# pangenome/poasta

Measured on AMD Instinct MI355X. Metric: Gcells/sec (aligned bases/sec in config), gap-affine POA alignment, 1k-node POA x 10k x 1 kbp queries per GPU, higher is better.
Workload: dtype u16

## Files before the change

include/poasta_amd.h:

```cpp
#ifndef POASTA_AMD_H
#define POASTA_AMD_H

#include <stdint.h>

#ifdef __cplusplus
extern "C" {
#endif

#define POA_NONE 0xFFFFFFFFu
#define POA_SCORE_UNVISITED 0xFFFFFFFFu

#define POA_OK 0
#define POA_ERR_INVALID_ARG (-1)
#define POA_ERR_NOT_A_DAG (-2)
#define POA_ERR_NO_DEVICE (-3)
#define POA_ERR_HIP (-4)
#define POA_ERR_CAPACITY (-5)
#define POA_ERR_OUT_OF_MEMORY (-6)
#define POA_ERR_UNSUPPORTED (-7)

#define POA_FLAG_AMBIGUOUS 0x01u
#define POA_FLAG_START_QUIRK 0x02u
#define POA_FLAG_REF_PANIC 0x04u
#define POA_FLAG_SHORT_QUERY 0x08u
// ... 175 lines not shown
#define POA_LAYOUT_DERIVED_GAPS 8u
#define POA_LAYOUT_RELATIVE 4u
int poa_batch_last_layout(poa_batch_t* b, uint32_t* layout);
int poa_batch_band_info(poa_batch_t* b, uint32_t out[4]);
enum {
    POA_KERNEL_NONE = 0,
    POA_KERNEL_FORWARD,
    POA_KERNEL_PACKED,
    POA_KERNEL_PX,
    POA_KERNEL_PXMW,
    POA_KERNEL_BAND
};
#define POA_LAUNCH_FUSE 1u
#define POA_LAUNCH_MW 2u
int poa_batch_last_launch(poa_batch_t* b, uint32_t chunk, uint32_t out[8]);
int poa_batch_band_pair_info(poa_batch_t* b, uint32_t out[4]);
#define POA_BAND_PAIR_MASK 3
#define POA_BAND_PAIR_RULE 2
#define POA_BAND_NARROW_SHIFT 2
int poa_batch_band_narrow_info(poa_batch_t* b, uint32_t out[4]);
int poa_batch_fetch_planes(poa_batch_t* b, uint32_t query, uint32_t* m, uint32_t* i, uint32_t* d);
int poa_batch_fetch_compact(poa_batch_t* b, uint32_t query, uint16_t* m_raw, uint16_t* d, uint8_t* d_kept);
int poa_batch_fetch_planes_2piece(poa_batch_t* b, uint32_t query, uint32_t* m, uint32_t* i1, uint32_t* d1, uint32_t* i2, uint32_t* d2);
void poa_batch_destroy(poa_batch_t* b);

typedef struct poa_multi poa_multi_t;
int poa_multi_footprint(const poa_graph_t* const* graphs, uint32_t n_graphs, const uint64_t* graph_qoff,
                        const uint64_t* qoff, const poa_config_t* cfg, uint64_t* bytes, uint64_t* largest_query_bytes);
int poa_multi_create(const poa_graph_t* const* graphs, uint32_t n_graphs, const uint64_t* graph_qoff, int device,
                     const uint8_t* qseq, const uint64_t* qoff, const poa_config_t* cfg, uint64_t workspace_bytes,
                     poa_multi_t** out);
int poa_multi_run(poa_multi_t* m, const poa_costs_t* costs, const poa_config_t* cfg, void* stream);
int poa_multi_fetch(poa_multi_t* m, uint32_t* score, poa_aln_pair_t* pairs, uint64_t* pair_off, uint64_t pair_capacity,
                    uint32_t* flags, poa_stats_t* stats);
int poa_multi_stats(poa_multi_t* m, poa_stats_t* stats);
int poa_multi_device_results(poa_multi_t* m, void** score, void** flags, void** pair_off, void** pairs);
int poa_multi_workspace_bytes(poa_multi_t* m, uint64_t* bytes);
void poa_multi_destroy(poa_multi_t* m);
int poa_align_multi(const poa_graph_t* const* graphs, uint32_t n_graphs, const uint64_t* graph_qoff,
                    const poa_costs_t* costs, const poa_config_t* cfg, const uint8_t* qseq, const uint64_t* qoff,
                    uint32_t* score, poa_aln_pair_t* pairs, uint64_t* pair_off, uint64_t pair_capacity, uint32_t* flags,
                    poa_stats_t* stats, int device);

int poa_multi_footprint_2piece(const poa_graph_t* const* graphs, uint32_t n_graphs, const uint64_t* graph_qoff,
                               const uint64_t* qoff, const poa_config_t* cfg, uint64_t* bytes, uint64_t* largest_query_bytes);
int poa_multi_create_2piece(const poa_graph_t* const* graphs, uint32_t n_graphs, const uint64_t* graph_qoff, int device,
                            const uint8_t* qseq, const uint64_t* qoff, const poa_config_t* cfg, uint64_t workspace_bytes,
                            poa_multi_t** out);
int poa_multi_run_2piece(poa_multi_t* m, const poa_costs2_t* costs, const poa_config_t* cfg, void* stream);
int poa_align_multi_2piece(const poa_graph_t* const* graphs, uint32_t n_graphs, const uint64_t* graph_qoff,
                           const poa_costs2_t* costs, const poa_config_t* cfg, const uint8_t* qseq, const uint64_t* qoff,
                           uint32_t* score, poa_aln_pair_t* pairs, uint64_t* pair_off, uint64_t pair_capacity,
                           uint32_t* flags, poa_stats_t* stats, int device);

typedef struct poa_scoreset poa_scoreset_t;
int poa_scoreset_footprint(const poa_graph_t* const* graphs, uint32_t n_graphs, uint32_t n_queries, const uint64_t* qoff,
                           uint64_t n_pairs, const uint32_t* pair_query, const uint32_t* pair_graph, const poa_config_t* cfg,
                           uint64_t* bytes, uint64_t* largest_pair_bytes);
int poa_scoreset_create(const poa_graph_t* const* graphs, uint32_t n_graphs, int device, uint32_t n_queries, const uint8_t* qseq,
                        const uint64_t* qoff, uint64_t n_pairs, const uint32_t* pair_query, const uint32_t* pair_graph,
                        const poa_config_t* cfg, uint64_t workspace_bytes, poa_scoreset_t** out);
int poa_scoreset_run(poa_scoreset_t* s, const poa_costs_t* costs, const poa_config_t* cfg, void* stream);
int poa_scoreset_run_2piece(poa_scoreset_t* s, const poa_costs2_t* costs, const poa_config_t* cfg, void* stream);
int poa_scoreset_fetch(poa_scoreset_t* s, uint32_t* score, uint32_t* flags, poa_stats_t* stats);
int poa_scoreset_stats(poa_scoreset_t* s, poa_stats_t* stats);
int poa_scoreset_device_results(poa_scoreset_t* s, void** score, void** flags);
int poa_scoreset_workspace_bytes(poa_scoreset_t* s, uint64_t* bytes);
void poa_scoreset_destroy(poa_scoreset_t* s);
int poa_score_pairs(const poa_graph_t* const* graphs, uint32_t n_graphs, const poa_costs_t* costs, const poa_config_t* cfg,
                    uint32_t n_queries, const uint8_t* qseq, const uint64_t* qoff, uint64_t n_pairs, const uint32_t* pair_query,
                    const uint32_t* pair_graph, uint32_t* score, uint32_t* flags, poa_stats_t* stats, int device);
int poa_score_pairs_2piece(const poa_graph_t* const* graphs, uint32_t n_graphs, const poa_costs2_t* costs, const poa_config_t* cfg,
                           uint32_t n_queries, const uint8_t* qseq, const uint64_t* qoff, uint64_t n_pairs,
                           const uint32_t* pair_query, const uint32_t* pair_graph, uint32_t* score, uint32_t* flags,
                           poa_stats_t* stats, int device);

#ifdef __cplusplus
}
#endif
#include "poasta_amd_scoreset_cap.h"
#include "poasta_amd_scoreset_best.h"
#include "poasta_amd_tb.h"
#include "poasta_amd_multi_dense.h"
#endif
```

poasta_amd/_lib.py:

```python
import ctypes as C
import os
import subprocess

_HERE = os.path.dirname(os.path.abspath(__file__))
LIB_PATH = os.environ.get("POA_LIB_PATH") or os.path.join(_HERE, "libpoasta_amd.so")
CSRC = os.path.join(_HERE, "csrc")

POA_OK = 0
ERRORS = {-1: "POA_ERR_INVALID_ARG", -2: "POA_ERR_NOT_A_DAG", -3: "POA_ERR_NO_DEVICE", -4: "POA_ERR_HIP",
          -5: "POA_ERR_CAPACITY", -6: "POA_ERR_OUT_OF_MEMORY", -7: "POA_ERR_UNSUPPORTED"}
POA_NONE = 0xFFFFFFFF
FLAG_AMBIGUOUS, FLAG_START_QUIRK, FLAG_REF_PANIC, FLAG_SHORT_QUERY, FLAG_TRUNCATED, FLAG_EMPTY_GRAPH = 1, 2, 4, 8, 16, 32
FLAG_CAPPED = 0x80

EXPORTS = ["poa_version", "poa_last_error", "poa_device_count", "poa_graph_create", "poa_graph_destroy",
           "poa_graph_rows", "poa_graph_node_rows", "poa_graph_update", "poa_align_batch", "poa_align_batch_ex", "poa_align_batch_2piece", "poa_align_batch_2piece_ex", "poa_planes_2piece", "poa_release_cache", "poa_batch_create", "poa_batch_run",
           "poa_batch_run_ex",
           "poa_batch_fetch", "poa_batch_stats", "poa_batch_device_results", "poa_batch_fetch_search_counters", "poa_batch_last_layout", "poa_batch_band_info", "poa_batch_band_pair_info", "poa_batch_band_narrow_info", "poa_batch_last_launch", "poa_batch_fetch_planes", "poa_batch_fetch_compact", "poa_batch_destroy",
           "poa_batch_run_2piece", "poa_batch_fetch_planes_2piece",
           "poa_graph_sweep_slots", "poa_batch_create_ex", "poa_batch_workspace_bytes", "poa_graph_checkpoint_plan", "poa_graph_checkpoint_plan2",
           "poa_multi_footprint", "poa_multi_create", "poa_multi_run", "poa_multi_fetch", "poa_multi_stats", "poa_multi_device_results",
           "poa_multi_workspace_bytes", "poa_multi_destroy", "poa_align_multi",
           "poa_multi_footprint_2piece", "poa_multi_create_2piece", "poa_multi_run_2piece", "poa_align_multi_2piece",
           "poa_scoreset_footprint", "poa_scoreset_create", "poa_scoreset_run", "poa_scoreset_run_2piece", "poa_scoreset_fetch",
           "poa_scoreset_stats", "poa_scoreset_device_results", "poa_scoreset_workspace_bytes", "poa_scoreset_destroy",
           "poa_score_pairs", "poa_score_pairs_2piece",
           "poa_graph_sweep_checks"]
EXPORTS_SCORESET_CAP = ["poa_scoreset_run_capped", "poa_scoreset_run_2piece_capped", "poa_scoreset_fetch_swept"]
EXPORTS_SCORESET_BEST = ["poa_scoreset_run_best", "poa_scoreset_run_2piece_best", "poa_scoreset_fetch_best", "poa_scoreset_device_best",
                         "poa_score_best", "poa_score_best_2piece"]
CFG_BEST_PAIR_ORDER = 2
EXPORTS_TB = ["poa_batch_tb_info"]
TB_LEAN_SHIFT = 4
EXPORTS_MULTI_DENSE = ["poa_multi_footprint_dense", "poa_multi_create_dense", "poa_multi_run_dense", "poa_align_multi_dense",
                       "poa_graph_compact_elems", "poa_multi_last_launch"]


class PoaBest(C.Structure):
    _fields_ = [("pair", C.c_uint32), ("score", C.c_uint32), ("flags", C.c_uint32), ("second_score", C.c_uint32),
                ("n_within", C.c_uint32), ("reserved", C.c_uint32 * 3)]


class PoaCosts2(C.Structure):
    _fields_ = [("mismatch", C.c_uint8), ("gap_open1", C.c_uint8), ("gap_extend1", C.c_uint8), ("gap_open2", C.c_uint8),
                ("gap_extend2", C.c_uint8), ("wide_planes", C.c_uint8), ("reserved", C.c_uint8 * 2)]


class PoaCosts(C.Structure):
    _fields_ = [("mismatch", C.c_uint8), ("gap_open", C.c_uint8), ("gap_extend", C.c_uint8), ("reserved", C.c_uint8)]


class PoaBound(C.Structure):
    _fields_ = [("kind", C.c_uint32), ("value", C.c_uint32)]


class PoaConfig(C.Structure):
    _fields_ = [("mode", C.c_uint32), ("heuristic", C.c_uint32), ("pruning", C.c_uint32), ("queue_entries_per_cell", C.c_float),
                ("flags", C.c_uint32), ("span", C.c_uint32), ("qry_free_begin", PoaBound), ("qry_free_end", PoaBound),
                ("graph_free_begin", PoaBound), ("graph_free_end", PoaBound), ("tune", C.c_uint32 * 32)]


TUNE_KEYS = ("PLANES", "COMPACT", "PACKED", "RELATIVE", "PX", "MF", "MW", "PXMW", "FWD_QUADS", "FUSE_TB", "TB_GROUP", "TB_DEPTH",
             "EXACT_IMPL", "EXACT_LANES", "EXACT_LDS", "WS_LANES", "WS_GROUP", "WS_WAVES", "WS_RING_GLOBAL", "WS_STATIC",
             "WS_CHUNK_CAP", "WS_PROF", "PS_LANES", "PS_LEAN", "TIMING", "WS_ADAPT", "WS_REC", "CKPT_ROWS", "BAND", "BAND_DELTA", "BAND_PAIR", "CAP_STRIDE")
EXACT_IMPLS = {"lane": 1, "wave": 2, "flat": 3}


def tune_from_env(cfg=None, **overrides):
    vals = {}
    for i, k in enumerate(TUNE_KEYS):
        v = overrides.get(k.lower(), os.environ.get("POA_" + k))
        if v is None or v == "":
            continue
        vals[i] = EXACT_IMPLS[v] if (k == "EXACT_IMPL" and v in EXACT_IMPLS) else int(v)
    nv = overrides.get("band_narrow", os.environ.get("POA_BAND_NARROW"))
    if nv is not None and nv != "":
        i = TUNE_KEYS.index("BAND_PAIR")
        vals[i] = (min(vals[i], 1) if i in vals else 2) | ((2 if int(nv) else 1) << 2)
    lv = overrides.get("tb_lean", os.environ.get("POA_TB_LEAN"))
    if lv is not None and lv != "":
        i = TUNE_KEYS.index("BAND_PAIR")
        vals[i] = (vals[i] if i in vals else 2) | ((2 if int(lv) else 1) << TB_LEAN_SHIFT)
    if cfg is None:
        if not vals:
            return None
        cfg = PoaConfig()
    for i, v in vals.items():
        cfg.tune[i] = v + 1
    return cfg


BOUND_UNBOUNDED, BOUND_INCLUDED, BOUND_EXCLUDED = 0, 1, 2
SPAN_GLOBAL, SPAN_ENDS_FREE = 0, 1


MODE_DENSE, MODE_EXACT, MODE_HYBRID, MODE_SCORE, MODE_CHECKPOINT, MODE_CHECKPOINT2 = 0, 1, 2, 3, 4, 5
HEURISTIC_DIJKSTRA, HEURISTIC_MINGAP = 0, 1
FLAG_EXACT_OVERFLOW = 0x40
CFG_FULL_PLANES = 1


class PoaStats(C.Structure):
    _fields_ = [("cells", C.c_uint64), ("bases", C.c_uint64), ("plane_bytes", C.c_uint64), ("n_queries", C.c_uint32),
                ("n_chunks", C.c_uint32), ("n_forward_launches", C.c_uint32), ("n_flagged", C.c_uint32),
                ("ms_forward", C.c_float), ("ms_traceback", C.c_float), ("ms_h2d", C.c_float), ("ms_d2h", C.c_float),
                ("ms_exact", C.c_float), ("n_exact", C.c_uint32), ("ms_total", C.c_float), ("n_runs", C.c_uint32)]

    def as_dict(self):
        return {k: getattr(self, k) for k, _ in self._fields_ }


class PoaError(RuntimeError):
    def __init__(self, code, msg):
        super().__init__("%s (%d): %s" % (ERRORS.get(code, "POA_ERR"), code, msg))
        self.code = code


def build(force=False):
    srcs = [os.path.join(CSRC, f) for f in os.listdir(CSRC)] + [os.path.join(_HERE, "..", "include", h) for h in ("poasta_amd.h", "poasta_amd_scoreset_cap.h", "poasta_amd_scoreset_best.h", "poasta_amd_tb.h", "poasta_amd_multi_dense.h")]
    stale = not os.path.exists(LIB_PATH) or any(os.path.getmtime(s) > os.path.getmtime(LIB_PATH) for s in srcs)
    if force or stale:
        subprocess.check_call(["make", "-C", CSRC] + (["-B"] if force else []))
    return LIB_PATH


_lib = None


def lib():
    global _lib
    if _lib is not None:
        return _lib
    if not os.path.exists(LIB_PATH):
        raise ImportError("poasta_amd: %s is missing — build it with `python -c 'import __graft_entry__ as g; g.build()'` "
                          "(hipcc --offload-arch=gfx950). There is no CPU fallback." % LIB_PATH)
    L = C.CDLL(LIB_PATH)
    vp = C.c_void_p
    L.poa_version.restype = C.c_char_p
    L.poa_last_error.restype = C.c_char_p
    L.poa_device_count.restype = C.c_int
    L.poa_graph_create.restype = C.c_int
    L.poa_graph_create.argtypes = [C.c_uint32, C.c_uint32, C.c_uint32, vp, vp, vp, vp, vp, C.POINTER(vp)]
    L.poa_graph_destroy.argtypes = [vp]
    L.poa_graph_destroy.restype = None
    L.poa_graph_rows.restype = C.c_uint32
    L.poa_graph_rows.argtypes = [vp]
    L.poa_graph_node_rows.restype = C.c_int
    L.poa_graph_node_rows.argtypes = [vp, vp]
    L.poa_align_batch.restype = C.c_int
    L.poa_align_batch.argtypes = [vp, C.POINTER(PoaCosts), C.c_uint32, vp, vp, vp, vp, vp, C.c_uint64, vp,
                                  C.POINTER(PoaStats), C.c_int]
    L.poa_align_batch_ex.restype = C.c_int
    L.poa_align_batch_ex.argtypes = [vp, C.POINTER(PoaCosts), C.POINTER(PoaConfig), C.c_uint32, vp, vp, vp, vp, vp, C.c_uint64, vp,
                                     C.POINTER(PoaStats), C.c_int]
    L.poa_align_batch_2piece.restype = C.c_int
    L.poa_align_batch_2piece.argtypes = [vp, C.POINTER(PoaCosts2), C.c_uint32, vp, vp, vp, vp, vp, C.c_uint64, vp,
                                         C.POINTER(PoaStats), C.c_int]
    L.poa_align_batch_2piece_ex.restype = C.c_int
    L.poa_align_batch_2piece_ex.argtypes = [vp, C.POINTER(PoaCosts2), C.POINTER(PoaConfig), C.c_uint32, vp, vp, vp, vp, vp, C.c_uint64, vp,
                                            C.POINTER(PoaStats), vp, C.c_int]
    L.poa_planes_2piece.restype = C.c_int
    L.poa_planes_2piece.argtypes = [vp, C.POINTER(PoaCosts2), vp, C.c_uint32, vp, vp, vp, vp, vp, C.c_int]
    L.poa_batch_run_ex.restype = C.c_int
    L.poa_batch_run_ex.argtypes = [vp, C.POINTER(PoaCosts), C.POINTER(PoaConfig), vp]
    L.poa_batch_create.restype = C.c_int
    L.poa_batch_create.argtypes = [vp, C.c_int, C.c_uint32, vp, vp, C.c_uint64, C.POINTER(vp)]
    L.poa_graph_sweep_slots.restype = C.c_int
    L.poa_graph_sweep_slots.argtypes = [vp, vp, vp]
    if hasattr(L, "poa_graph_sweep_checks"):
        L.poa_graph_sweep_checks.restype = C.c_int
        L.poa_graph_sweep_checks.argtypes = [vp, C.c_uint32, vp, vp]
        L.poa_scoreset_run_capped.restype = C.c_int
        L.poa_scoreset_run_capped.argtypes = [vp, C.POINTER(PoaCosts), C.POINTER(PoaConfig), vp, vp]
        L.poa_scoreset_run_2piece_capped.restype = C.c_int
        L.poa_scoreset_run_2piece_capped.argtypes = [vp, C.POINTER(PoaCosts2), C.POINTER(PoaConfig), vp, vp]
        L.poa_scoreset_fetch_swept.restype = C.c_int
        L.poa_scoreset_fetch_swept.argtypes = [vp, vp]
    if hasattr(L, "poa_scoreset_run_best"):
        L.poa_scoreset_run_best.restype = C.c_int
        L.poa_scoreset_run_best.argtypes = [vp, C.POINTER(PoaCosts), C.POINTER(PoaConfig), C.c_uint32, vp, vp]
        L.poa_scoreset_run_2piece_best.restype = C.c_int
        L.poa_scoreset_run_2piece_best.argtypes = [vp, C.POINTER(PoaCosts2), C.POINTER(PoaConfig), C.c_uint32, vp, vp]
        L.poa_scoreset_fetch_best.restype = C.c_int
        L.poa_scoreset_fetch_best.argtypes = [vp, vp]
        L.poa_scoreset_device_best.restype = C.c_int
        L.poa_scoreset_device_best.argtypes = [vp, C.POINTER(vp)]
        L.poa_score_best.restype = C.c_int
        L.poa_score_best.argtypes = [vp, C.c_uint32, C.POINTER(PoaCosts), C.POINTER(PoaConfig), C.c_uint32, vp, vp, C.c_uint64, vp, vp,
                                     C.c_uint32, vp, vp, vp, vp, C.POINTER(PoaStats), C.c_int]
        L.poa_score_best_2piece.restype = C.c_int
        L.poa_score_best_2piece.argtypes = [vp, C.c_uint32, C.POINTER(PoaCosts2), C.POINTER(PoaConfig), C.c_uint32, vp, vp, C.c_uint64, vp, vp,
                                            C.c_uint32, vp, vp, vp, vp, C.POINTER(PoaStats), C.c_int]
    L.poa_graph_checkpoint_plan.restype = C.c_int
    L.poa_graph_checkpoint_plan.argtypes = [vp, C.c_uint32, vp, vp, vp]
    L.poa_graph_checkpoint_plan2.restype = C.c_int
    L.poa_graph_checkpoint_plan2.argtypes = [vp, C.c_uint32, vp, vp, vp]
    L.poa_batch_create_ex.restype = C.c_int
    L.poa_batch_create_ex.argtypes = [vp, C.c_int, C.c_uint32, vp, vp, C.POINTER(PoaConfig), C.c_uint64, C.POINTER(vp)]
    L.poa_batch_workspace_bytes.restype = C.c_int
    L.poa_batch_workspace_bytes.argtypes = [vp, C.POINTER(C.c_uint64)]
    L.poa_batch_run.restype = C.c_int
    L.poa_batch_run.argtypes = [vp, C.POINTER(PoaCosts), vp]
    L.poa_batch_fetch.restype = C.c_int
    L.poa_batch_fetch.argtypes = [vp, vp, vp, vp, C.c_uint64, vp, C.POINTER(PoaStats)]
    L.poa_batch_stats.restype = C.c_int
    L.poa_batch_stats.argtypes = [vp, C.POINTER(PoaStats)]
    L.poa_batch_fetch_search_counters.restype = C.c_int
    L.poa_batch_fetch_search_counters.argtypes = [vp, vp]
    L.poa_batch_last_layout.restype = C.c_int
    L.poa_batch_last_layout.argtypes = [vp, vp]
    if hasattr(L, "poa_batch_band_info"):
        L.poa_batch_band_info.restype = C.c_int
        L.poa_batch_band_info.argtypes = [vp, vp]
    if hasattr(L, "poa_batch_band_pair_info"):
        L.poa_batch_band_pair_info.restype = C.c_int
        L.poa_batch_band_pair_info.argtypes = [vp, vp]
    if hasattr(L, "poa_batch_band_narrow_info"):
        L.poa_batch_band_narrow_info.restype = C.c_int
        L.poa_batch_band_narrow_info.argtypes = [vp, vp]
    if hasattr(L, "poa_batch_tb_info"):
        L.poa_batch_tb_info.restype = C.c_int
        L.poa_batch_tb_info.argtypes = [vp, vp]
    if hasattr(L, "poa_batch_last_launch"):
        L.poa_batch_last_launch.restype = C.c_int
        L.poa_batch_last_launch.argtypes = [vp, C.c_uint32, vp]
    L.poa_batch_device_results.restype = C.c_int
    L.poa_batch_device_results.argtypes = [vp, C.POINTER(vp), C.POINTER(vp), C.POINTER(vp), C.POINTER(vp)]
    L.poa_batch_fetch_planes.restype = C.c_int
    L.poa_batch_fetch_planes.argtypes = [vp, C.c_uint32, vp, vp, vp]
    if hasattr(L, "poa_batch_fetch_compact"):
        L.poa_batch_fetch_compact.restype = C.c_int
        L.poa_batch_fetch_compact.argtypes = [vp, C.c_uint32, vp, vp, vp]
    L.poa_batch_run_2piece.restype = C.c_int
    L.poa_batch_run_2piece.argtypes = [vp, C.POINTER(PoaCosts2), C.POINTER(PoaConfig), vp]
    L.poa_batch_fetch_planes_2piece.restype = C.c_int
    L.poa_batch_fetch_planes_2piece.argtypes = [vp, C.c_uint32, vp, vp, vp, vp, vp]
    L.poa_batch_destroy.argtypes = [vp]
    L.poa_batch_destroy.restype = None
    L.poa_multi_footprint.restype = C.c_int
    L.poa_multi_footprint.argtypes = [vp, C.c_uint32, vp, vp, C.POINTER(PoaConfig), C.POINTER(C.c_uint64), C.POINTER(C.c_uint64)]
    L.poa_multi_create.restype = C.c_int
    L.poa_multi_create.argtypes = [vp, C.c_uint32, vp, C.c_int, vp, vp, C.POINTER(PoaConfig), C.c_uint64, C.POINTER(vp)]
    L.poa_multi_run.restype = C.c_int
    L.poa_multi_run.argtypes = [vp, C.POINTER(PoaCosts), C.POINTER(PoaConfig), vp]
    L.poa_multi_fetch.restype = C.c_int
    L.poa_multi_fetch.argtypes = [vp, vp, vp, vp, C.c_uint64, vp, C.POINTER(PoaStats)]
    L.poa_multi_stats.restype = C.c_int
    L.poa_multi_stats.argtypes = [vp, C.POINTER(PoaStats)]
    L.poa_multi_device_results.restype = C.c_int
    L.poa_multi_device_results.argtypes = [vp, C.POINTER(vp), C.POINTER(vp), C.POINTER(vp), C.POINTER(vp)]
    L.poa_multi_workspace_bytes.restype = C.c_int
    L.poa_multi_workspace_bytes.argtypes = [vp, C.POINTER(C.c_uint64)]
    L.poa_multi_destroy.argtypes = [vp]
    L.poa_multi_destroy.restype = None
    L.poa_align_multi.restype = C.c_int
    L.poa_align_multi.argtypes = [vp, C.c_uint32, vp, C.POINTER(PoaCosts), C.POINTER(PoaConfig), vp, vp, vp, vp, vp, C.c_uint64, vp,
                                  C.POINTER(PoaStats), C.c_int]
    L.poa_multi_footprint_2piece.restype = C.c_int
    L.poa_multi_footprint_2piece.argtypes = L.poa_multi_footprint.argtypes
    L.poa_multi_create_2piece.restype = C.c_int
    L.poa_multi_create_2piece.argtypes = L.poa_multi_create.argtypes
    L.poa_multi_run_2piece.restype = C.c_int
    L.poa_multi_run_2piece.argtypes = [vp, C.POINTER(PoaCosts2), C.POINTER(PoaConfig), vp]
    L.poa_align_multi_2piece.restype = C.c_int
    L.poa_align_multi_2piece.argtypes = [vp, C.c_uint32, vp, C.POINTER(PoaCosts2), C.POINTER(PoaConfig), vp, vp, vp, vp, vp, C.c_uint64, vp,
                                         C.POINTER(PoaStats), C.c_int]
    if hasattr(L, "poa_multi_create_dense"):
        L.poa_multi_footprint_dense.restype = C.c_int
        L.poa_multi_footprint_dense.argtypes = L.poa_multi_footprint.argtypes
        L.poa_multi_create_dense.restype = C.c_int
        L.poa_multi_create_dense.argtypes = L.poa_multi_create.argtypes
        L.poa_multi_run_dense.restype = C.c_int
        L.poa_multi_run_dense.argtypes = L.poa_multi_run.argtypes
        L.poa_align_multi_dense.restype = C.c_int
        L.poa_align_multi_dense.argtypes = L.poa_align_multi.argtypes
        L.poa_graph_compact_elems.restype = C.c_int
        L.poa_graph_compact_elems.argtypes = [vp, C.c_uint32, C.POINTER(C.c_uint64)]
        L.poa_multi_last_launch.restype = C.c_int
        L.poa_multi_last_launch.argtypes = [vp, C.c_uint32, vp]
    L.poa_scoreset_footprint.restype = C.c_int
    L.poa_scoreset_footprint.argtypes = [vp, C.c_uint32, C.c_uint32, vp, C.c_uint64, vp, vp, C.POINTER(PoaConfig), C.POINTER(C.c_uint64),
                                         C.POINTER(C.c_uint64)]
    L.poa_scoreset_create.restype = C.c_int
    L.poa_scoreset_create.argtypes = [vp, C.c_uint32, C.c_int, C.c_uint32, vp, vp, C.c_uint64, vp, vp, C.POINTER(PoaConfig), C.c_uint64,
                                      C.POINTER(vp)]
    L.poa_scoreset_run.restype = C.c_int
    L.poa_scoreset_run.argtypes = [vp, C.POINTER(PoaCosts), C.POINTER(PoaConfig), vp]
    L.poa_scoreset_run_2piece.restype = C.c_int
    L.poa_scoreset_run_2piece.argtypes = [vp, C.POINTER(PoaCosts2), C.POINTER(PoaConfig), vp]
    L.poa_scoreset_fetch.restype = C.c_int
    L.poa_scoreset_fetch.argtypes = [vp, vp, vp, C.POINTER(PoaStats)]
    L.poa_scoreset_stats.restype = C.c_int
    L.poa_scoreset_stats.argtypes = [vp, C.POINTER(PoaStats)]
    L.poa_scoreset_device_results.restype = C.c_int
    L.poa_scoreset_device_results.argtypes = [vp, C.POINTER(vp), C.POINTER(vp)]
    L.poa_scoreset_workspace_bytes.restype = C.c_int
    L.poa_scoreset_workspace_bytes.argtypes = [vp, C.POINTER(C.c_uint64)]
    L.poa_scoreset_destroy.argtypes = [vp]
    L.poa_scoreset_destroy.restype = None
    L.poa_score_pairs.restype = C.c_int
    L.poa_score_pairs.argtypes = [vp, C.c_uint32, C.POINTER(PoaCosts), C.POINTER(PoaConfig), C.c_uint32, vp, vp, C.c_uint64, vp, vp, vp, vp,
                                  C.POINTER(PoaStats), C.c_int]
    L.poa_score_pairs_2piece.restype = C.c_int
    L.poa_score_pairs_2piece.argtypes = [vp, C.c_uint32, C.POINTER(PoaCosts2), C.POINTER(PoaConfig), C.c_uint32, vp, vp, C.c_uint64, vp, vp,
                                         vp, vp, C.POINTER(PoaStats), C.c_int]
# ... 8 lines not shown
```

poasta_amd/aligner.py:

```python
import ctypes as C
import os

import numpy as np

from . import _lib
from .graph import FlatGraph, pack_queries


class GapAffine:

    def __init__(self, cost_mismatch, cost_gap_extend, cost_gap_open):
        for v in (cost_mismatch, cost_gap_extend, cost_gap_open):
            if not 0 <= int(v) <= 255:
                raise ValueError("GapAffine costs are u8")
        self.cost_mismatch, self.cost_gap_extend, self.cost_gap_open = int(cost_mismatch), int(cost_gap_extend), int(cost_gap_open)

    def mismatch(self):
        return self.cost_mismatch

    def gap_open(self):
        return self.cost_gap_open

    def gap_extend(self):
        return self.cost_gap_extend
# ... 250 lines not shown
        if isinstance(costs, GapAffine2Piece):
            _lib.check(_lib.lib().poa_batch_run_2piece(self.handle, C.byref(c), C.byref(config) if config is not None else None,
                                                       C.c_void_p(stream or 0)))
            return
        if config is None:
            config = _lib.tune_from_env()
        if config is None:
            _lib.check(_lib.lib().poa_batch_run(self.handle, C.byref(c), C.c_void_p(stream or 0)))
        else:
            _lib.check(_lib.lib().poa_batch_run_ex(self.handle, C.byref(c), C.byref(config), C.c_void_p(stream or 0)))

    def fetch(self, want_pairs=True, pinned=False, copy=False):
        n = self.n
        bufs = self._host_buffers(want_pairs, pinned)
        score, flags, pair_off, pairs = bufs
        st = _lib.PoaStats()
        _lib.check(_lib.lib().poa_batch_fetch(self.handle, _p(score), _p(pairs), _p(pair_off), self.pair_capacity,
                                              _p(flags), C.byref(st)))
        if want_pairs:
            pairs = pairs[:int(pair_off[n])]
        if copy and pinned:
            score, pairs, pair_off, flags = score.copy(), pairs.copy(), pair_off.copy(), flags.copy()
        return BatchResult(score, pairs, pair_off, flags, st.as_dict())

    def _host_buffers(self, want_pairs, pinned):
        n = self.n
        if pinned:
            cached = getattr(self, "_pinned", None)
            if cached is None:
                try:
                    import torch
                    mk = lambda shape, dt: torch.empty(shape, dtype=dt, pin_memory=True).numpy()
                    cached = (mk((n,), torch.int32).view(np.uint32), mk((n,), torch.int32).view(np.uint32),
                              mk((n + 1,), torch.int64).view(np.uint64), mk((max(self.pair_capacity, 1), 2), torch.int32).view(np.uint32))
                except Exception:
                    cached = False
                self._pinned = cached
            if cached:
                return cached[0], cached[1], cached[2], (cached[3] if want_pairs else None)
        score, flags = np.zeros(n, np.uint32), np.zeros(n, np.uint32)
        pair_off = np.zeros(n + 1, np.uint64)
        pairs = np.zeros((max(self.pair_capacity, 1), 2), np.uint32) if want_pairs else None
        return score, flags, pair_off, pairs

    def stats(self):
        st = _lib.PoaStats()
        _lib.check(_lib.lib().poa_batch_stats(self.handle, C.byref(st)))
        return st.as_dict()

    def workspace_bytes(self):
        v = C.c_uint64(0)
        _lib.check(_lib.lib().poa_batch_workspace_bytes(self.handle, C.byref(v)))
        return int(v.value)

    def search_counters(self):
        out = np.zeros((self.n, 4), np.uint32)
        _lib.check(_lib.lib().poa_batch_fetch_search_counters(self.handle, _p(out)))
        return out

    def layout(self):
        v = C.c_uint32(0)
        _lib.check(_lib.lib().poa_batch_last_layout(self.handle, C.byref(v)))
        return {name for bit, name in ((1, "u16"), (2, "compact"), (4, "relative"), (8, "derived_gaps")) if v.value & bit}

    def band_info(self):
        out = (C.c_uint32 * 4)()
        _lib.check(_lib.lib().poa_batch_band_info(self.handle, out))
        return {"used": bool(out[0]), "banded": int(out[1]), "fell_back": int(out[2]), "min_d": int(out[3])}

    def band_pair_info(self):
        out = (C.c_uint32 * 4)()
        _lib.check(_lib.lib().poa_batch_band_pair_info(self.handle, out))
        return {"paired": int(out[0]), "single": int(out[1]), "rule_count": int(out[2]), "ran_paired": bool(out[3])}

    def band_narrow_info(self):
        out = (C.c_uint32 * 4)()
        _lib.check(_lib.lib().poa_batch_band_narrow_info(self.handle, out))
        return {"ran": int(out[0]), "certified": int(out[1]), "certified_512": int(out[2]), "chosen_by": (None, "rule", "override")[int(out[3])]}

    def tb_info(self):
        out = (C.c_uint32 * 4)()
        _lib.check(_lib.lib().poa_batch_tb_info(self.handle, out))
        return {"kernel": (None, "generic", "lean")[int(out[0])], "lanes": int(out[1]), "depth": int(out[2]), "walks": int(out[3])}

    def launches(self):
        out = []
        while True:
            v = (C.c_uint32 * 8)()
            rc = _lib.lib().poa_batch_last_launch(self.handle, len(out), v)
            if rc == -1 and (out or self.n == 0):
                return out
            _lib.check(rc)
            out.append({"kernel": LAUNCH_KERNELS[v[0]], "quads": int(v[1]), "fuse": bool(v[2] & 1), "mw": bool(v[2] & 2),
                        "waves": int(v[3]), "code_fmt": int(v[4]), "tb_lanes": int(v[5]), "tb_depth": int(v[6]), "queries": int(v[7])})

    def device_results(self):
        ptrs = [C.c_void_p() for _ in range(4)]
        _lib.check(_lib.lib().poa_batch_device_results(self.handle, *[C.byref(p) for p in ptrs]))
        return dict(zip(("score", "flags", "pair_off", "pairs"), [p.value for p in ptrs]))

    def planes(self, query):
        rows = self.dg.graph.n
        cols = int(self.qoff[query + 1] - self.qoff[query]) + 1
        m, i, d = (np.zeros((rows, cols), np.uint32) for _ in range(3))
        _lib.check(_lib.lib().poa_batch_fetch_planes(self.handle, query, _p(m), _p(i), _p(d)))
        return m, i, d

    def compact_planes(self, query):
        rows = self.dg.graph.n
        cols = int(self.qoff[query + 1] - self.qoff[query]) + 1
        m_raw, d = np.zeros((rows, cols), np.uint16), np.zeros((rows, cols), np.uint16)
        kept = np.zeros(rows, np.uint8)
        _lib.check(_lib.lib().poa_batch_fetch_compact(self.handle, query, _p(m_raw), _p(d), _p(kept)))
        return m_raw, d, kept.astype(bool)

    def planes_2piece(self, query):
        rows = self.dg.graph.n
        cols = int(self.qoff[query + 1] - self.qoff[query]) + 1
        out = [np.zeros((rows, cols), np.uint32) for _ in range(5)]
        _lib.check(_lib.lib().poa_batch_fetch_planes_2piece(self.handle, query, *[_p(a) for a in out]))
        return out

    def close(self):
        if getattr(self, "handle", None):
            _lib.lib().poa_batch_destroy(self.handle)
            self.handle = None

    def __del__(self):
        try:
            self.close()
        except Exception:
            pass


class _MultiInput:

    def __init__(self, graphs, seqs_per_graph=None, graph_qoff=None, qseq=None, qoff=None):
        self.dgs = [_device_graph(g) for g in graphs]
        if seqs_per_graph is not None:
            if len(seqs_per_graph) != len(self.dgs):
                raise ValueError("seqs_per_graph needs one list of queries per graph")
            graph_qoff = np.concatenate([[0], np.cumsum([len(s) for s in seqs_per_graph])])
            qseq, qoff = pack_queries([q for s in seqs_per_graph for q in s])
        self.graph_qoff = np.ascontiguousarray(graph_qoff, np.uint64)
        self.qseq = np.ascontiguousarray(qseq, np.uint8)
        self.qoff = np.ascontiguousarray(qoff, np.uint64)
        self.n = len(self.qoff) - 1
        if len(self.graph_qoff) != len(self.dgs) + 1:
            raise ValueError("graph_qoff needs n_graphs + 1 entries")
        if int(self.graph_qoff[-1]) != self.n:
            raise ValueError("graph_qoff[n_graphs] = %d is not the query count %d" % (int(self.graph_qoff[-1]), self.n))
        self.handles = (C.c_void_p * max(len(self.dgs), 1))(*[dg.handle for dg in self.dgs])
        self.n_graphs = len(self.dgs)
        per_graph = np.diff(self.graph_qoff.astype(np.int64))
        self.pair_capacity = int(self.qoff[-1]) + int(sum(int(c) * dg.graph.n for c, dg in zip(per_graph, self.dgs) if c > 0))


def multi_footprint(graphs, seqs_per_graph=None, graph_qoff=None, qseq=None, qoff=None, config=None, two_piece=False, dense=False):
    if dense and two_piece:
        raise ValueError("multi_footprint: the dense multi-graph batch is one-piece")
    mi = _MultiInput(graphs, seqs_per_graph, graph_qoff, qseq, qoff)
    total, largest = C.c_uint64(0), C.c_uint64(0)
    fn = _lib.lib().poa_multi_footprint_2piece if two_piece else (_lib.lib().poa_multi_footprint_dense if dense else _lib.lib().poa_multi_footprint)
    _lib.check(fn(mi.handles, mi.n_graphs, _p(mi.graph_qoff), _p(mi.qoff), C.byref(config) if config is not None else None,
                  C.byref(total), C.byref(largest)))
    return int(total.value), int(largest.value)
# ... 380 lines not shown
```

poasta_amd/csrc/poa_dense_plan.cpp:

```cpp
#include "poa_dense_plan.hpp"

#include <algorithm>

namespace poa_amd {

uint64_t score_bound(uint64_t open, uint64_t extend, uint64_t n_open, uint64_t n_extend) { return open * n_open + extend * n_extend; }
bool u16_cells_suffice(uint64_t open, uint64_t extend, uint64_t n_open, uint64_t n_extend) {
    return score_bound(open, extend, n_open, n_extend) <= 65534;
}
bool planes32(const TuneView& T) { const int* pv = T.ptr(POA_TUNE_PLANES); return pv && *pv == 32; }

uint32_t mw_waves(uint32_t strips) {
    const uint32_t groups = (strips + DENSE_MW_MAX_WAVES - 1) / DENSE_MW_MAX_WAVES;
    return (strips + groups - 1) / groups;
}

bool pxmw_ok(const TuneView& T, uint32_t count, uint32_t max_pitch) {
    if (const int* v = T.ptr(POA_TUNE_PXMW)) return (*v) != 0;
    return (uint64_t)count * ((max_pitch + 1023) / 1024) >= 1024;
}

DenseRunPlan plan_dense_run(uint32_t gap_open, uint32_t gap_extend, uint64_t max_len, uint64_t min_path_nodes, uint32_t mode, bool want_full,
                            bool plan16_same, const TuneView& T) {
    DenseRunPlan R;
    R.ub = score_bound(gap_open, gap_extend, (max_len ? 1 : 0) + (min_path_nodes ? 1 : 0), max_len + min_path_nodes);
    R.narrow = R.ub <= 65534 && !planes32(T);
    R.compact = R.narrow && !want_full;
    if (const int* cv = T.ptr(POA_TUNE_COMPACT)) { if ((*cv) == 0) R.compact = false; }
    R.packed = true;
    if (const int* pv2 = T.ptr(POA_TUNE_PACKED)) R.packed = (*pv2) != 0;
    const uint64_t rel_ub = 2 * ((uint64_t)gap_open + (uint64_t)gap_extend * max_len);
    R.relative = !R.narrow && rel_ub <= 65534 && !want_full && R.packed && !T.ptr(POA_TUNE_PLANES) && !T.ptr(POA_TUNE_COMPACT);
    if (const int* rv = T.ptr(POA_TUNE_RELATIVE)) {
        if ((*rv) == 0) R.relative = false;
        else R.relative = rel_ub <= 65534 && !want_full && R.packed;
    }
    if (R.relative) { R.narrow = true; R.compact = true; }
    R.plan = (R.narrow && mode == POA_MODE_DENSE && !plan16_same) ? (R.compact ? 2 : 1) : 0;
    R.spec_depth = 12;
    if (const int* sv = T.ptr(POA_TUNE_TB_DEPTH)) { const int v = (*sv); if (v >= 1 && v <= 64) R.spec_depth = (uint32_t)v; }
    R.tb_group = 0;
    if (const int* gv = T.ptr(POA_TUNE_TB_GROUP)) { const int v = (*gv); if (v == 8 || v == 16 || v == 32 || v == 64) R.tb_group = v; }
    R.fuse_tb = false;
    if (const int* fv = T.ptr(POA_TUNE_FUSE_TB)) R.fuse_tb = (*fv) != 0;
    R.quads_override = 0;
    if (const int* ov = T.ptr(POA_TUNE_FWD_QUADS)) R.quads_override = (*ov);
    R.want_band = mode == POA_MODE_DENSE && gap_extend > 0;
    if (const int* bv = T.ptr(POA_TUNE_BAND)) R.want_band = R.want_band && (*bv) != 0;
    R.band_cap = 0xFFFFFFFFu;
    if (const int* dv = T.ptr(POA_TUNE_BAND_DELTA)) R.band_cap = (*dv) > 0 ? (uint32_t)(*dv) : 0u;
    R.band_pair = -1;
    R.band_narrow = -1;
    R.tb_lean = -1;
    if (const int* pv = T.ptr(POA_TUNE_BAND_PAIR)) {
        const int p = (*pv) & POA_BAND_PAIR_MASK, n = ((*pv) >> POA_BAND_NARROW_SHIFT) & 3, l = ((*pv) >> POA_TB_LEAN_SHIFT) & 3;
        if (p != POA_BAND_PAIR_RULE) R.band_pair = p != 0 ? 1 : 0;
        if (n) R.band_narrow = n - 1;
        if (l == 1 || l == 2) R.tb_lean = l - 1;
    }
    R.tb_lean_mode = mode == POA_MODE_DENSE;
    return R;
}

bool tb_lean_eligible(const DenseRunPlan& R, uint32_t tb_lanes, uint32_t code_fmt, uint64_t plane_elems) {
    return R.tb_lean_mode && tb_lanes != 0 && R.compact && code_fmt == 4 && !R.relative && plane_elems < (1ull << 32);
}

constexpr uint32_t BAND_NARROW_MIN_SHARE = 4;
uint32_t band_narrow_class(uint32_t d_n, uint32_t L) {
    if (d_n < 4) return 2;
    return (uint64_t)BAND_NARROW_MIN_SHARE * (d_n - 4) >= L ? 0 : 1;
}
uint32_t band_narrow_pairs(const DenseRunPlan& R, bool pair_by_rule, uint32_t n_rule, uint32_t n_any) {
    if (R.band_narrow == 0) return 0;
    if (R.band_narrow > 0) return n_any;
    return pair_by_rule ? n_rule : 0;
}

DenseChunkPlan plan_dense_chunk(const DenseRunPlan& R, uint32_t count, uint32_t max_pitch, const TuneView& T, uint64_t plane_elems) {
    uint32_t lk = POA_KERNEL_NONE, lq = 0, lwaves = 4, code_fmt = 0;
    bool lfuse = false, lmw = false;
    int mf = -1;
    const int quads_override = R.quads_override;
    if (R.narrow) {
        uint32_t quads = max_pitch <= 512 ? 1 : 2;
        if (quads_override == 1 || quads_override == 2) quads = (uint32_t)quads_override;
        if (R.relative) quads = 2;
        lk = R.compact && R.packed ? POA_KERNEL_PACKED : POA_KERNEL_FORWARD; lq = quads;
        if (R.compact && R.packed) {
            bool mw = max_pitch > 512 * quads;
            if (const int* mv = T.ptr(POA_TUNE_MW)) mw = mw && ((*mv) != 0 || R.relative);
            bool px = max_pitch <= 1024 && quads == 2 && (!R.fuse_tb || R.relative);
            if (const int* xv = T.ptr(POA_TUNE_PX)) px = (px && (*xv) != 0) || (px && R.relative);
            if (px) {
                mf = R.relative ? 0 : (R.ub <= 4094 ? 2 : (R.ub <= 16382 ? 1 : 0));
                if (const int* fv2 = T.ptr(POA_TUNE_MF)) mf = (*fv2) == 3 ? (mf >= 1 ? 3 : 0) : std::min(mf, std::max(0, (*fv2)));
                else if (mf >= 1) mf = 3;
                code_fmt = mf == 3 ? 4u : (mf == 2 ? 3u : (mf == 1 ? 2u : 1u));
                lk = (mf == 3 && R.want_band && max_pitch > 512) ? POA_KERNEL_BAND : POA_KERNEL_PX;
            } else if (mw && (R.relative || pxmw_ok(T, count, max_pitch))) {
                code_fmt = 1;
                lk = POA_KERNEL_PXMW; lq = 2; lmw = true; lwaves = mw_waves((max_pitch + 1023) / 1024);
            } else if (mw) {
                if (!quads_override) quads = ((uint64_t)count * ((max_pitch + 1023) / 1024) >= 8192) ? 2 : 1;
                lq = quads; lmw = true; lwaves = mw_waves((max_pitch + 512 * quads - 1) / (512 * quads));
            } else lfuse = R.fuse_tb;
        } else if (!R.compact) lfuse = R.fuse_tb;
    } else {
        uint32_t quads = max_pitch <= 256 ? 1 : (max_pitch <= 512 ? 2 : 4);
        if (quads_override == 1 || quads_override == 2 || quads_override == 4) quads = (uint32_t)quads_override;
        bool mw = max_pitch > 1024;
        if (const int* mv = T.ptr(POA_TUNE_MW)) mw = mw && (*mv) != 0;
        lk = POA_KERNEL_FORWARD; lq = quads;
        if (mw) {
            const uint32_t s2 = (max_pitch + 511) / 512, s4 = (max_pitch + 1023) / 1024;
            const uint32_t g2 = (s2 + DENSE_MW_MAX_WAVES - 1) / DENSE_MW_MAX_WAVES, g4 = (s4 + 9) / 10;
            bool wide = 14 * g4 < 10 * g2 || (uint64_t)count * s4 >= 8192;
            if (quads_override == 4) wide = true;
            if (quads_override == 2) wide = false;
            lq = wide ? 4 : 2; lmw = true; lwaves = wide ? (s4 + g4 - 1) / g4 : (s2 + g2 - 1) / g2;
        } else lfuse = R.fuse_tb;
    }
    uint32_t ltb = 0, ldepth = R.spec_depth;
    if (!(R.fuse_tb && !R.relative && max_pitch <= 1024 && (!R.compact || R.packed))) {
        const int tbg = R.tb_group ? R.tb_group : (count <= 6144 ? 64 : (count <= 12288 ? 32 : 16));
        ltb = R.compact ? (uint32_t)tbg : 64u;
        if (R.compact && !T.ptr(POA_TUNE_TB_DEPTH)) ldepth = tbg == 16 ? 16u : 32u;
    }
    const bool lean = R.tb_lean != 0 && tb_lean_eligible(R, ltb, code_fmt, plane_elems);
    return {{lk, lq, (lfuse ? POA_LAUNCH_FUSE : 0u) | (lmw ? POA_LAUNCH_MW : 0u), lwaves, code_fmt, ltb, ldepth, count}, mf, lk == POA_KERNEL_BAND, ltb != 0, lean};
}

}
```

poasta_amd/csrc/poa_dense_plan.hpp:

```cpp
#pragma once
#include <cstdint>

#include "../../include/poasta_amd.h"

struct TuneView {
    int val[POA_TUNE_COUNT]; bool set[POA_TUNE_COUNT];
    explicit TuneView(const poa_config_t* cfg) { for (int k = 0; k < POA_TUNE_COUNT; ++k) { set[k] = cfg && cfg->tune[k] != 0; val[k] = set[k] ? (int)cfg->tune[k] - 1 : 0; } }
    const int* ptr(int k) const { return set[k] ? &val[k] : nullptr; }
};

namespace poa_amd {
constexpr uint32_t DENSE_MW_MAX_WAVES = 16;
uint64_t score_bound(uint64_t open, uint64_t extend, uint64_t n_open, uint64_t n_extend);
bool u16_cells_suffice(uint64_t open, uint64_t extend, uint64_t n_open, uint64_t n_extend);
bool planes32(const TuneView& T);
uint32_t mw_waves(uint32_t strips);
bool pxmw_ok(const TuneView& T, uint32_t count, uint32_t max_pitch);

struct DenseRunPlan {
    uint64_t ub;
    bool narrow, compact, relative, packed;
    int plan;
    bool fuse_tb, want_band;
    int quads_override, band_pair, tb_group;
    int band_narrow;
    uint32_t band_cap, spec_depth;
    int tb_lean;
    bool tb_lean_mode;
};
DenseRunPlan plan_dense_run(uint32_t gap_open, uint32_t gap_extend, uint64_t max_len, uint64_t min_path_nodes, uint32_t mode, bool full_planes,
                            bool plan16_same, const TuneView& T);

struct DenseChunkPlan {
    uint32_t v[8];
    int mf;
    bool band;
    bool separate_tb;
    bool lean_tb;
};
DenseChunkPlan plan_dense_chunk(const DenseRunPlan& R, uint32_t count, uint32_t max_pitch, const TuneView& T, uint64_t plane_elems = ~0ull);
bool tb_lean_eligible(const DenseRunPlan& R, uint32_t tb_lanes, uint32_t code_fmt, uint64_t plane_elems);
uint32_t band_narrow_class(uint32_t d_n, uint32_t L);
uint32_t band_narrow_pairs(const DenseRunPlan& R, bool pair_by_rule, uint32_t n_rule, uint32_t n_any);
}
```

poasta_amd/csrc/poa_engine.hip:

```cpp
#include <hip/hip_runtime.h>

#include <algorithm>
#include <array>
#include <chrono>
#include <cstdio>
#include <cstdlib>
#include <cstring>
#include <map>
#include <memory>
#include <new>
#include <mutex>
#include <string>
#include <vector>

#include "../../include/poasta_amd.h"
#include "poa_graph.hpp"
#include "poa_exact_kernel.hpp"
#include "poa_wsearch.hpp"
#include "poa_fsearch.hpp"

#include "poa_dense_plan.hpp"
#include "poa_kernels.hpp"
#include "poa_traceback_mf.hpp"
#include "poa_forward_packed.hpp"
#include "poa_forward_px.hpp"
#include "poa_band_plan.hpp"
#include "poa_forward_band.hpp"
#include "poa_twopiece.hpp"
#include "poa_sweep_rows.hpp"
#include "poa_forward_sweep.hpp"
#include "poa_checkpoint.hpp"
#include "poa_checkpoint2.hpp"
#include "poa_multi_plan.hpp"
#include "poa_multi.hpp"
#include "poa_multi_dense.hpp"
#include "poa_scoreset_plan.hpp"
#include "poa_scoreset.hpp"

using namespace poa_amd;

namespace {
thread_local std::string g_err;

int fail(int code, const std::string& msg) {
    g_err = msg;
    return code;
}
#define HIP_TRY(expr)                                                                              \
    do {                                                                                           \
        hipError_t _e = (expr);                                                                    \
        if (_e != hipSuccess)                                                                      \
            return fail(POA_ERR_HIP, std::string(#expr) + ": " + hipGetErrorString(_e));           \
    } while (0)

struct BufCache {
    static constexpr size_t kMaxCachedBytes = 8ull << 30;
    std::mutex mu;
    std::multimap<size_t, void*> free_blocks[16];
    size_t cached_bytes[16] = {};
    void* take(int dev, size_t need, size_t* got) {
        if (dev < 0 || dev >= 16) return nullptr;
        std::lock_guard<std::mutex> lk(mu);
        auto it = free_blocks[dev].lower_bound(need);
        if (it == free_blocks[dev].end() || it->first > 2 * need + (1u << 20)) return nullptr;
        void* p = it->second;
        *got = it->first;
        cached_bytes[dev] -= it->first;
        free_blocks[dev].erase(it);
        return p;
    }
    bool give(int dev, void* p, size_t bytes) {
        if (dev < 0 || dev >= 16) return false;
        std::lock_guard<std::mutex> lk(mu);
        if (cached_bytes[dev] + bytes > kMaxCachedBytes) return false;
        free_blocks[dev].emplace(bytes, p);
        cached_bytes[dev] += bytes;
        return true;
    }
    void release_all() {
        std::lock_guard<std::mutex> lk(mu);
        for (int d = 0; d < 16; ++d) {
            if (free_blocks[d].empty()) continue;
            (void)hipSetDevice(d);
            for (auto& kv : free_blocks[d]) (void)hipFree(kv.second);
            free_blocks[d].clear();
            cached_bytes[d] = 0;
        }
    }
};
static BufCache g_buf_cache;

template <typename T>
struct DevBuf {
    T* p = nullptr;
    size_t n = 0;
    size_t cap_bytes = 0;
    int dev = -1;
    ~DevBuf() { drop(); }
    void drop() {
        if (!p) return;
        if (!g_buf_cache.give(dev, p, cap_bytes)) { (void)hipSetDevice(dev); (void)hipFree(p); }
        p = nullptr; cap_bytes = 0;
    }
    hipError_t alloc(size_t count) {
// ... 62 lines not shown
    FlatGraph g;
    SweepRows sweep;
    CheckpointPlan ckpt;
    CheckpointPlan ckpt2;
    std::mutex bubble_mu;
};

struct poa_batch {
    const poa_graph* graph = nullptr;
    int device = 0;
    uint32_t n_queries = 0;
    uint64_t total_bases = 0, total_cells = 0, plane_bytes_total = 0;
    std::vector<uint64_t> h_qoff;
    std::vector<uint32_t> h_pitch;
    std::vector<uint64_t> h_scratch_off;
    struct Chunk { uint32_t first, count; };
    struct Plan {
        std::vector<Chunk> chunks;
        std::vector<uint64_t> off;
        uint32_t max_chunk = 0;
        DevBuf<uint64_t> d_off;
    };
    Plan plan[4];
    uint64_t plan_ws = 0;
    bool two_piece = false;
    bool plan16_same = true;
    int active_plan = 0;
    const Plan& cur() const { return plan[active_plan]; }
    uint64_t max_len = 0;
    bool narrow = false;
    bool compact = false;
    int cols_per_lane = 16;

    DevBuf<RowMeta> d_rows;
    DevBuf<uint32_t> d_pred_rows;
    DevBuf<uint32_t> d_row_depth, d_pred_k;
    DevBuf<uint32_t> d_dslot, d_pred_dslot;
    bool relative = false;
    bool dense_narrow = false, dense_compact = false, dense_relative = false, dense_derived_gaps = false;
    DevBuf<uint8_t> d_qseq;
    DevBuf<uint64_t> d_qoff, d_scratch_off, d_pair_off;
    DevBuf<uint32_t> d_pitch, d_carry, d_score, d_flags, d_npairs;
    PlaneWorkspace d_planes;
    DevBuf<uint2> d_scratch, d_pairs;
    DevBuf<uint32_t> d_succ_off, d_succ_rows, d_dist_min, d_dist_max, d_nbm_off, d_ex_status, d_exit_idx, d_ex_head, d_node_row, d_sp_to_end, d_ex_end;
    DevBuf<FlatGraph::NodeBubble> d_nbm;
    DevBuf<uint8_t> d_ex_sym;
    DevBuf<uint64_t> d_ex_reached, d_ex_rsum;
    DevBuf<ExQEntry> d_ex_pool;
    DevBuf<ExStackEntry> d_ex_stack;
    uint32_t ex_n_prio = 0, ex_pool_cap = 0, ex_stack_cap = 0, ex_wpn = 0, ex_swpn = 0;
    uint32_t ex_win = 64;
    uint32_t ex_skew = 0;
    DevBuf<uint32_t> d_ex_order;
    DevBuf<uint32_t> d_pipeline_error;
    DevBuf<unsigned long long> d_ex_prof;
    DevBuf<uint32_t> d_ex_counters;
    DevBuf<uint32_t> d_ex_logs;
    DevBuf<FlatGraph::RowRec> d_ex_rec;
    bool exact_ready = false;
    bool prof_on = false;
    uint32_t last_mode = 0;
    bool sweep = false;
    uint32_t sweep_slots = 1;
    uint64_t sweep_slotted = 0;
    uint64_t sweep_bytes_written = 0;
    bool ckpt = false;
    CheckpointPlan ckpt_plan;
    uint32_t ckpt_slots = 0;
    bool ckpt2 = false;
    DevBuf<uint32_t> d_ck_snap_off, d_ck_snap_dst, d_ck_pred_src, d_ck_boundary;

    bool band_ready = false;
    uint32_t band_n_seg = 0;
    std::vector<uint32_t> h_band_cls, h_band_d;
    DevBuf<uint32_t> d_band_cls, d_band_d, d_band_base;
    DevBuf<uint32_t> d_band_list, d_band_count;
    std::vector<uint32_t> h_band_dn;
    DevBuf<uint32_t> d_band_dn, d_band_base_n, d_band_list_n;
    std::vector<uint32_t> h_band_order;
    std::vector<uint32_t> h_band_nnarrow_rule, h_band_nnarrow_any;
    uint32_t narrow_ran = 0, narrow_how = 0, narrow_chunks = 0;
    uint32_t tb_kernel = 0, tb_lanes = 0, tb_depth = 0, tb_walks = 0;
    int band_pair_plan = -1;
    std::vector<uint32_t> h_band_npair;
    DevBuf<uint32_t> d_band_order;
    uint32_t pair_paired = 0, pair_single = 0;
    bool band_used = false;
    uint32_t band_queries = 0, band_min_d = 0, band_chunks = 0;
    std::vector<DenseChunkPlan> launches;

    std::vector<std::vector<hipEvent_t>> runs;
    std::vector<std::vector<hipEvent_t>> free_sets;
    bool ran = false;
    hipStream_t last_stream = nullptr;
    float ms_h2d = 0.f;

    ~poa_batch() {
        for (auto& r : runs) for (auto e : r) (void)hipEventDestroy(e);
        for (auto& r : free_sets) for (auto e : r) (void)hipEventDestroy(e);
    }
};

static int check_pipeline_error(poa_batch* b) {
    uint32_t w = 0;
    HIP_TRY(hipMemcpy(&w, b->d_pipeline_error.p, 4, hipMemcpyDeviceToHost));
    if (w) {
        (void)hipMemset(b->d_pipeline_error.p, 0, 4);
        return fail(POA_ERR_HIP, "multi-wave forward pipeline timed out waiting for a neighbouring strip: results discarded");
    }
    return POA_OK;
}

static void collect_stats(poa_batch* b, poa_stats_t* stats) {
    const uint32_t n = b->n_queries;
    const uint32_t keep_flagged = stats->n_flagged;
    stats->cells = b->total_cells; stats->bases = b->total_bases; stats->plane_bytes = (b->sweep || b->ckpt) ? b->sweep_bytes_written : (b->two_piece ? b->total_cells * 5 * (b->narrow ? 2 : 4) : b->plane_bytes_total);
    stats->n_queries = n; stats->n_chunks = (uint32_t)b->cur().chunks.size();
    stats->n_flagged = keep_flagged;
    stats->ms_h2d = b->ms_h2d; stats->ms_d2h = 0.f;
    float fwd = 0.f, tb = 0.f, ex = 0.f, total = 0.f;
    uint32_t launches = 0;
    for (auto& events : b->runs) {
        if (n) {
            size_t ev = 1;
            hipEvent_t prev = events[0];
            const size_t n_chunks = (events.size() - 2) / 3;
            for (size_t c = 0; c < n_chunks; ++c) {
                float a = 0.f, t2 = 0.f, t3 = 0.f;
                (void)hipEventElapsedTime(&a, prev, events[ev]);
                (void)hipEventElapsedTime(&t2, events[ev], events[ev + 1]);
                (void)hipEventElapsedTime(&t3, events[ev + 1], events[ev + 2]);
                fwd += a; tb += t2; ex += t3;
                prev = events[ev + 2];
                ev += 3;
                launches++;
            }
            float tail = 0.f, tot = 0.f;
            (void)hipEventElapsedTime(&tail, prev, events[ev]);
            tb += tail;
            (void)hipEventElapsedTime(&tot, events[0], events[ev]);
            total += tot;
        }
    }
    stats->n_runs = (uint32_t)b->runs.size();
    stats->n_forward_launches = launches;
    if (b->sweep) tb = 0.f;
    stats->ms_forward = fwd; stats->ms_traceback = tb; stats->ms_exact = ex; stats->ms_total = total;
    for (auto& r : b->runs) b->free_sets.push_back(std::move(r));
    b->runs.clear();
}

struct RunFrame {
    poa_batch* b = nullptr;
    hipStream_t stream = nullptr;
    std::vector<hipEvent_t> events;
    size_t ev = 1;

    int open(poa_batch* batch, const std::string& refusal) {
        b = batch;
        if (b->runs.size() >= 256) return fail(POA_ERR_UNSUPPORTED, refusal);
        return POA_OK;
    }
    int begin(hipStream_t s, size_t n_chunks) {
        stream = s;
        b->last_stream = stream;
// ... 207 lines not shown
        hipLaunchKernelGGL(poa_forward_pxmw_kernel, grid, block, 0, stream, fp);
        break;
    case POA_KERNEL_PACKED:
        if (mw && quads == 1) hipLaunchKernelGGL((poa_forward_packed_kernel<1, false, true>), grid, block, 0, stream, fp, tp);
        else if (mw) hipLaunchKernelGGL((poa_forward_packed_kernel<2, false, true>), grid, block, 0, stream, fp, tp);
        else if (quads == 1 && fuse) hipLaunchKernelGGL((poa_forward_packed_kernel<1, true, false>), grid, block, 0, stream, fp, tp);
        else if (quads == 1) hipLaunchKernelGGL((poa_forward_packed_kernel<1, false, false>), grid, block, 0, stream, fp, tp);
        else if (fuse) hipLaunchKernelGGL((poa_forward_packed_kernel<2, true, false>), grid, block, 0, stream, fp, tp);
        else hipLaunchKernelGGL((poa_forward_packed_kernel<2, false, false>), grid, block, 0, stream, fp, tp);
        break;
    default:
        if (mw && quads == 4) hipLaunchKernelGGL((poa_forward_kernel<4, uint32_t, false, false, true>), grid, block, 0, stream, fp, tp);
        else if (mw) hipLaunchKernelGGL((poa_forward_kernel<2, uint32_t, false, false, true>), grid, block, 0, stream, fp, tp);
        else if (R.compact && quads == 1) hipLaunchKernelGGL((poa_forward_kernel<1, uint16_t, false, true>), grid, block, 0, stream, fp, tp);
        else if (R.compact) hipLaunchKernelGGL((poa_forward_kernel<2, uint16_t, false, true>), grid, block, 0, stream, fp, tp);
        else if (R.narrow && quads == 1) plain(uint16_t{}, integral_constant<int, 1>{});
        else if (R.narrow) plain(uint16_t{}, integral_constant<int, 2>{});
        else if (quads == 1) plain(uint32_t{}, integral_constant<int, 1>{});
        else if (quads == 2) plain(uint32_t{}, integral_constant<int, 2>{});
        else plain(uint32_t{}, integral_constant<int, 4>{});
    }
}

int launch_band(poa_batch* b, size_t ci, const DenseRunPlan& R, const FwdParams& fp, hipStream_t stream) {
    const poa_batch::Chunk& ch = b->cur().chunks[ci];
    const uint32_t blocks = (ch.count + 3) / 4;
    if (const int rc = prepare_band(b)) return rc;
    BandParams bp;
    bp.cls = b->d_band_cls.p; bp.cls_d = b->d_band_d.p; bp.cls_base = b->d_band_base.p; bp.n_seg = b->band_n_seg;
    bp.d_cap = R.band_cap; bp.list = b->d_band_list.p; bp.count = b->d_band_count.p + ci; bp.order = nullptr;
    bp.n_order = nullptr; bp.count_nf = nullptr;
    const size_t n_chunks = b->cur().chunks.size();
    uint32_t n_pairs = 0, n_narrow = 0;
    if (R.band_pair != 0) {
        if (const int rc = prepare_band_pairs(b)) return rc;
        n_pairs = b->h_band_npair[ci];
        const bool by_rule = band_pair_rule(2 * n_pairs);
        if (R.band_pair < 0 && !by_rule) n_pairs = 0;
        if (n_pairs) n_narrow = band_narrow_pairs(R, by_rule, b->h_band_nnarrow_rule[ci], b->h_band_nnarrow_any[ci]);
    }
    if (n_pairs) {
        const uint32_t n_single = ch.count - 2 * n_pairs;
        FwdParams fq = fp;
        BandParams bq = bp;
        if (n_narrow) {
            BandParams bn = bp;
            bn.cls_d = b->d_band_dn.p; bn.cls_base = b->d_band_base_n.p;
            bn.list = b->d_band_list_n.p; bn.count = b->d_band_count.p + n_chunks + ci;
            fq.n_queries = n_narrow; bn.order = b->d_band_order.p + ch.first;
            hipLaunchKernelGGL(poa_forward_band2_kernel<6>, dim3((n_narrow + 3) / 4), dim3(256), 0, stream, fq, bn);
            HIP_TRY(hipGetLastError());
            fq.n_queries = 2 * n_narrow; bq.order = b->d_band_list_n.p + fp.first_query;
            bq.n_order = bn.count; bq.count_nf = b->d_band_count.p + 2 * n_chunks + ci;
            hipLaunchKernelGGL((poa_forward_band_kernel<false, true>), dim3((2 * n_narrow + 3) / 4), dim3(256), 0, stream, fq, bq);
            HIP_TRY(hipGetLastError());
            bq.n_order = nullptr; bq.count_nf = nullptr;
            b->narrow_ran += 2 * n_narrow; b->narrow_chunks = (uint32_t)ci + 1;
            b->narrow_how = R.band_narrow > 0 ? 2u : 1u;
        }
        if (n_pairs > n_narrow) {
            fq.n_queries = n_pairs - n_narrow; bq.order = b->d_band_order.p + ch.first + 2 * n_narrow;
            hipLaunchKernelGGL(poa_forward_band2_kernel<8>, dim3((n_pairs - n_narrow + 3) / 4), dim3(256), 0, stream, fq, bq);
        }
        if (n_single) {
            HIP_TRY(hipGetLastError());
            fq.n_queries = n_single; bq.order = b->d_band_order.p + ch.first + 2 * n_pairs;
            hipLaunchKernelGGL((poa_forward_band_kernel<false, true>), dim3((n_single + 3) / 4), dim3(256), 0, stream, fq, bq);
        }
        b->pair_paired += 2 * n_pairs; b->pair_single += n_single;
    } else {
        hipLaunchKernelGGL(poa_forward_band_kernel<false>, dim3(blocks), dim3(256), 0, stream, fp, bp);
        b->pair_single += ch.count;
    }
    HIP_TRY(hipGetLastError());
    hipLaunchKernelGGL(poa_forward_band_kernel<true>, dim3(blocks), dim3(256), 0, stream, fp, bp);
    uint32_t min_d = 0xFFFFFFFFu;
    for (uint32_t i = ch.first; i < ch.first + ch.count; ++i) min_d = std::min(min_d, std::min(b->h_band_d[b->h_band_cls[i]], R.band_cap));
    for (uint32_t k = 0; k < 2 * n_narrow; ++k) min_d = std::min(min_d, std::min(b->h_band_dn[b->h_band_cls[b->h_band_order[ch.first + k]]], R.band_cap));
    b->band_min_d = b->band_used ? std::min(b->band_min_d, min_d) : min_d;
    b->band_used = true; b->band_queries += ch.count; b->band_chunks = (uint32_t)ci + 1;
    return POA_OK;
}

void launch_traceback(const DenseRunPlan& R, const DenseChunkPlan& c, const TbParams& tp, hipStream_t stream) {
    const uint32_t lanes = c.v[5], per_block = 256 / lanes;
    const dim3 grid((c.v[7] + per_block - 1) / per_block), block(256);
    TbParams tpg = tp;
    tpg.spec_depth = c.v[6];
    if (c.lean_tb && lanes == 16) hipLaunchKernelGGL((poa_traceback_mf_kernel<16>), grid, block, 0, stream, tpg);
    else if (c.lean_tb && lanes == 32) hipLaunchKernelGGL((poa_traceback_mf_kernel<32>), grid, block, 0, stream, tpg);
    else if (c.lean_tb && lanes == 8) hipLaunchKernelGGL((poa_traceback_mf_kernel<8>), grid, block, 0, stream, tpg);
    else if (c.lean_tb) hipLaunchKernelGGL((poa_traceback_mf_kernel<64>), grid, block, 0, stream, tpg);
    else if (R.compact && lanes == 16) hipLaunchKernelGGL((poa_traceback_kernel<uint16_t, true, 16>), grid, block, 0, stream, tpg);
    else if (R.compact && lanes == 32) hipLaunchKernelGGL((poa_traceback_kernel<uint16_t, true, 32>), grid, block, 0, stream, tpg);
    else if (R.compact && lanes == 8) hipLaunchKernelGGL((poa_traceback_kernel<uint16_t, true, 8>), grid, block, 0, stream, tpg);
    else if (R.compact) hipLaunchKernelGGL((poa_traceback_kernel<uint16_t, true>), grid, block, 0, stream, tpg);
    else if (R.narrow) hipLaunchKernelGGL((poa_traceback_kernel<uint16_t, false>), grid, block, 0, stream, tp);
    else hipLaunchKernelGGL((poa_traceback_kernel<uint32_t, false>), grid, block, 0, stream, tp);
}

template <typename SearchParams>
void fill_search_params(SearchParams& sp, poa_batch* b, const ExactParams& ep, const TuneView& T) {
    sp.E = ep;
    sp.chunks = reinterpret_cast<ExU4*>(b->d_ex_pool.p);
    sp.chunk_cap = b->ex_pool_cap / BQ_CHUNK;
    if (const int* cv = T.ptr(POA_TUNE_WS_CHUNK_CAP)) { const int v = (*cv); if (v >= 1 && (uint32_t)v < sp.chunk_cap) sp.chunk_cap = (uint32_t)v; }
    sp.win = b->ex_win;
    sp.counters = b->d_ex_counters.p;
    sp.prof = T.ptr(POA_TUNE_WS_PROF) ? b->d_ex_prof.p : nullptr;
    sp.work_counter = nullptr; sp.order = nullptr;
}

uint32_t resident_blocks(poa_batch* b, const void* kfn, uint32_t wpb, uint32_t lds_bytes) {
    int per_cu = 1, cus = 256;
    (void)hipDeviceGetAttribute(&cus, hipDeviceAttributeMultiprocessorCount, b->device);
    if (hipOccupancyMaxActiveBlocksPerMultiprocessor(&per_cu, kfn, (int)(64 * wpb), lds_bytes) != hipSuccess || per_cu < 1) per_cu = 1;
    return (uint32_t)cus * (uint32_t)per_cu;
}

template <typename SearchParams>
int persistent_schedule(poa_batch* b, const poa_batch::Chunk& ch, uint32_t resident, hipStream_t stream, SearchParams& sp, uint32_t& n_blocks) {
    std::vector<uint32_t> sc(ch.count), ord(ch.count);
    HIP_TRY(hipMemcpyAsync(sc.data(), b->d_score.p + ch.first, (size_t)ch.count * 4, hipMemcpyDeviceToHost, stream));
    HIP_TRY(hipStreamSynchronize(stream));
    for (uint32_t i = 0; i < ch.count; ++i) ord[i] = i;
    std::stable_sort(ord.begin(), ord.end(), [&](uint32_t a, uint32_t c2) { return sc[a] > sc[c2]; });
    HIP_TRY(b->d_ex_order.alloc(ch.count + 1));
    HIP_TRY(hipMemcpyAsync(b->d_ex_order.p + 1, ord.data(), (size_t)ch.count * 4, hipMemcpyHostToDevice, stream));
    HIP_TRY(hipMemsetAsync(b->d_ex_order.p, 0, 4, stream));
    HIP_TRY(hipStreamSynchronize(stream));
    sp.work_counter = b->d_ex_order.p; sp.order = b->d_ex_order.p + 1;
    n_blocks = resident;
    return POA_OK;
}

int replay_flat(poa_batch* b, const poa_batch::Chunk& ch, const ExactParams& ep, const TuneView& T, bool ends_free, int lds_cap, hipStream_t stream) {
    const FlatGraph& fg = b->graph->g;
    const uint32_t win = b->ex_win, graph_lds = exact_lds_bytes(fg.n, ep.n_succ, ep.n_nbm);
    FSearchParams pp;
    fill_search_params(pp, b, ep, T);
    pp.max_lanes = 63;
    if (const int* lv = T.ptr(POA_TUNE_PS_LANES)) { const int v = (*lv); if (v >= 1 && v <= 63) pp.max_lanes = (uint32_t)v; }
    pp.lean = (!fg.row_rec.empty() && !ends_free) ? 1u : 0u;
    if (const int* lv = T.ptr(POA_TUNE_PS_LEAN)) pp.lean = (pp.lean && (*lv) != 0) ? 1u : 0u;
    const uint32_t group = pp.lean ? 8u : 16u;
    const uint32_t qpw = 64 / group;
    pp.group = group;
    if (pp.max_lanes > group) pp.max_lanes = group;
    const uint64_t lds_budget = std::min<uint64_t>((uint64_t)lds_cap, 160u * 1024u);
    const uint64_t ring_b = ((uint64_t)qpw * 3 * win * 4 + 15) & ~15ull;
    const uint64_t rec_b = pp.lean ? ((sizeof(FlatGraph::RowRec) * (uint64_t)fg.n + 15) & ~15ull) : 0;
    const uint64_t stage_b = pp.lean ? rec_b : graph_lds;
    bool ring_lds = ring_b + ps_lds_bytes() <= lds_budget && !T.ptr(POA_TUNE_WS_RING_GLOBAL);
    uint64_t per_wave = (ring_lds ? ring_b : 0) + ps_lds_bytes();
    bool stage = stage_b + per_wave <= lds_budget;
    if (const int* gv = T.ptr(POA_TUNE_EXACT_LDS)) stage = stage && (*gv) != 0;
    uint32_t wpb = (uint32_t)std::min<uint64_t>(8, (lds_budget - (stage ? stage_b : 0)) / per_wave);
    if (const int* wv = T.ptr(POA_TUNE_WS_WAVES)) { const int v = (*wv); if (v >= 1 && (uint32_t)v <= wpb) wpb = (uint32_t)v; }
    if (wpb < 1) return fail(POA_ERR_UNSUPPORTED, "exact replay: the step's logs do not fit the LDS");
    pp.graph_lds = (stage && !pp.lean) ? graph_lds : 0;
    pp.rec_lds = (stage && pp.lean) ? (uint32_t)rec_b : 0;
    pp.waves_per_block = wpb;
    pp.ring_global = ring_lds ? nullptr : b->d_ex_head.p;
    const uint32_t lds_bytes = pp.graph_lds + pp.rec_lds + (uint32_t)(wpb * per_wave);
    const void* kfn = pp.lean ? reinterpret_cast<const void*>(poa_fsearch_lean_kernel) : reinterpret_cast<const void*>(poa_fsearch_kernel);
    if (lds_bytes > 48u * 1024u) HIP_TRY(hipFuncSetAttribute(kfn, hipFuncAttributeMaxDynamicSharedMemorySize, (int)lds_bytes));
    const uint32_t per_block = wpb * qpw;
    uint32_t n_blocks = (ch.count + per_block - 1) / per_block;
    const uint32_t resident = resident_blocks(b, kfn, wpb, lds_bytes);
    if (n_blocks > resident && !T.ptr(POA_TUNE_WS_STATIC)) {
        if (const int rc = persistent_schedule(b, ch, resident, stream, pp, n_blocks)) return rc;
    }
// ... 296 lines not shown
    if (ndev <= 0) return fail(POA_ERR_NO_DEVICE, "no HIP device visible: the gfx950 path has no CPU fallback");
    if (device < 0 || device >= ndev) return fail(POA_ERR_INVALID_ARG, "poa_batch_create: device ordinal out of range");
    HIP_TRY(hipSetDevice(device));

    std::unique_ptr<poa_batch> b(new (std::nothrow) poa_batch);
    if (!b) return fail(POA_ERR_OUT_OF_MEMORY, "host allocation failed");
    const FlatGraph& fg = g->g;
    b->graph = g; b->device = device; b->n_queries = n_queries;
    const uint32_t rows = fg.n;
    b->sweep = sweep;
    b->sweep_slots = std::max<uint32_t>(g->sweep.n_slots, 1u);
    b->sweep_slotted = g->sweep.n_slotted;
    b->ckpt = ckpt;
    b->ckpt2 = ckpt2;
    b->ckpt_slots = g->sweep.n_slots;
    try {
        if (ckpt) {
            const CheckpointPlan& own = ckpt2 ? g->ckpt2 : g->ckpt;
            if (ckpt_rows == 0 || ckpt_rows == own.segment_rows) b->ckpt_plan = own;
            else build_checkpoint_plan(fg, g->sweep, ckpt_rows, b->ckpt_plan, ckpt2);
        }
        b->h_qoff.assign(qoff, qoff + n_queries + 1);
        b->h_pitch.resize(n_queries);
        b->h_scratch_off.resize((size_t)n_queries + 1);
    } catch (const std::bad_alloc&) { return fail(POA_ERR_OUT_OF_MEMORY, "host allocation failed"); }

    uint64_t scratch_total = 0, max_len = 0;
    std::vector<uint64_t> q_plane_elems(n_queries);
    for (uint32_t i = 0; i < n_queries; ++i) {
        const uint64_t L = qoff[i + 1] - qoff[i];
        max_len = std::max(max_len, L);
        const uint32_t pitch = (uint32_t)(((L + 1 + 63) / 64) * 64);
        b->h_pitch[i] = pitch;
        q_plane_elems[i] = sweep ? 2ull * b->sweep_slots * pitch : (ckpt ? (uint64_t)b->ckpt_plan.rows_per_query * pitch : 3ull * rows * pitch);
        b->h_scratch_off[i] = scratch_total;
        if (!sweep) scratch_total += L + rows;
        b->max_len = std::max<uint64_t>(b->max_len, L);
        b->total_bases += L;
        b->total_cells += (uint64_t)rows * (L + 1);
        b->plane_bytes_total += q_plane_elems[i] * 4;
    }
    b->h_scratch_off[n_queries] = scratch_total;

    size_t free_b = 0, total_b = 0;
    HIP_TRY(hipMemGetInfo(&free_b, &total_b));
    const bool sweep_carry = (sweep || ckpt) && max_len + 1 > 1024;
    const uint64_t carry_words = ckpt2 ? 6 : 4;
    const uint64_t fixed = scratch_total * 16 + (uint64_t)n_queries * 64 + qoff[n_queries] + (64ull << 20) +
                           (sweep_carry ? 4ull * carry_words * n_queries * rows : 0);
    uint64_t ws = workspace_bytes;
    if (ws == 0) {
        const uint64_t avail = free_b > fixed ? (uint64_t)((free_b - fixed) * 0.85) : 0;
        ws = std::min<uint64_t>(b->plane_bytes_total, avail);
    }
    if (sweep || ckpt) ws = std::min<uint64_t>(ws, b->plane_bytes_total);
    uint64_t biggest = 0;
    for (uint32_t i = 0; i < n_queries; ++i) biggest = std::max(biggest, q_plane_elems[i] * 4);
    if (ws < biggest) {
        if (workspace_bytes == 0 || workspace_bytes < biggest) {
            if (biggest + fixed > free_b)
                return fail(POA_ERR_OUT_OF_MEMORY, "score planes of the largest query do not fit in device memory");
            ws = biggest;
        }
    }
    auto make_plan = [&](poa_batch::Plan& pl, uint64_t elem_bytes, bool compact_size) {
        build_chunk_plan(pl, n_queries, ws, elem_bytes, [&](uint32_t i) {
            return compact_size ? compact_plane_elems(rows, b->h_pitch[i], fg.n_store_d) : q_plane_elems[i];
        });
    };
    b->plan_ws = ws;
    make_plan(b->plan[0], 4, false);
    b->plan16_same = sweep || b->plan[0].chunks.size() <= 1;
    if (!b->plan16_same) { make_plan(b->plan[1], 2, false); make_plan(b->plan[2], 2, !ckpt); }
    const uint32_t max_chunk_any = std::max(b->plan[0].max_chunk, std::max(b->plan[1].max_chunk, b->plan[2].max_chunk));
    b->cols_per_lane = 16;

    HIP_TRY(b->d_rows.alloc(fg.rows.size()));
    HIP_TRY(b->d_pred_rows.alloc(std::max<size_t>(fg.pred_rows.size(), 1)));
    HIP_TRY(b->d_pred_k.alloc(std::max<size_t>(fg.pred_k.size(), 1)));
    HIP_TRY(b->d_row_depth.alloc(std::max<size_t>(fg.row_depth.size(), 1)));
    const bool sweep_tables = sweep || ckpt;
    HIP_TRY(b->d_dslot.alloc(std::max<size_t>(sweep_tables ? g->sweep.slot.size() : fg.d_slot.size(), 1)));
    HIP_TRY(b->d_pred_dslot.alloc(std::max<size_t>(sweep_tables ? g->sweep.pred_slot.size() : fg.pred_dslot.size(), 1)));
    if (ckpt) {
        const CheckpointPlan& cp = b->ckpt_plan;
        HIP_TRY(b->d_ck_snap_off.alloc(cp.snap_off.size()));
        HIP_TRY(b->d_ck_snap_dst.alloc(std::max<size_t>(cp.snap_dst.size(), 1)));
        HIP_TRY(b->d_ck_pred_src.alloc(std::max<size_t>(cp.pred_src.size(), 1)));
        HIP_TRY(b->d_ck_boundary.alloc(cp.boundary.size()));
        HIP_TRY(hipMemcpy(b->d_ck_snap_off.p, cp.snap_off.data(), cp.snap_off.size() * 4, hipMemcpyHostToDevice));
        if (!cp.snap_dst.empty()) HIP_TRY(hipMemcpy(b->d_ck_snap_dst.p, cp.snap_dst.data(), cp.snap_dst.size() * 4, hipMemcpyHostToDevice));
        if (!cp.pred_src.empty()) HIP_TRY(hipMemcpy(b->d_ck_pred_src.p, cp.pred_src.data(), cp.pred_src.size() * 4, hipMemcpyHostToDevice));
        HIP_TRY(hipMemcpy(b->d_ck_boundary.p, cp.boundary.data(), cp.boundary.size() * 4, hipMemcpyHostToDevice));
    }
    HIP_TRY(b->d_qseq.alloc(std::max<uint64_t>(qoff[n_queries], 1)));
    HIP_TRY(b->d_qoff.alloc((size_t)n_queries + 1));
    HIP_TRY(b->d_pitch.alloc(std::max<uint32_t>(n_queries, 1)));
    for (int k = 0; k < (b->plan16_same ? 1 : 3); ++k) HIP_TRY(b->plan[k].d_off.alloc(std::max<uint32_t>(n_queries, 1)));
    HIP_TRY(b->d_scratch_off.alloc((size_t)n_queries + 1));
    HIP_TRY(b->d_pair_off.alloc((size_t)n_queries + 1));
    HIP_TRY(b->d_score.alloc(std::max<uint32_t>(n_queries, 1)));
    HIP_TRY(b->d_flags.alloc(std::max<uint32_t>(n_queries, 1)));
    HIP_TRY(b->d_npairs.alloc(std::max<uint32_t>(n_queries, 1)));
    HIP_TRY(b->d_scratch.alloc(std::max<uint64_t>(scratch_total, 1)));
    HIP_TRY(b->d_pairs.alloc(std::max<uint64_t>(scratch_total, 1)));
    HIP_TRY(b->d_carry.alloc(std::max<uint64_t>((sweep_tables ? (sweep_carry ? carry_words : 0ull) : 2ull) * max_chunk_any * rows, 1)));
    HIP_TRY(b->d_pipeline_error.alloc(1));
    HIP_TRY(hipMemset(b->d_pipeline_error.p, 0, 4));
    if (n_queries) {
        std::string werr;
        if (!b->d_planes.acquire(device, ws + 256, werr, sweep_tables)) return fail(POA_ERR_OUT_OF_MEMORY, "score-plane workspace: " + werr);
    }

    hipEvent_t e0, e1;
    HIP_TRY(hipEventCreate(&e0));
    HIP_TRY(hipEventCreate(&e1));
    HIP_TRY(hipEventRecord(e0, nullptr));
    HIP_TRY(hipMemcpy(b->d_rows.p, fg.rows.data(), fg.rows.size() * sizeof(RowMeta), hipMemcpyHostToDevice));
    if (!fg.pred_rows.empty())
        HIP_TRY(hipMemcpy(b->d_pred_rows.p, fg.pred_rows.data(), fg.pred_rows.size() * 4, hipMemcpyHostToDevice));
    if (!fg.pred_k.empty())
        HIP_TRY(hipMemcpy(b->d_pred_k.p, fg.pred_k.data(), fg.pred_k.size() * 4, hipMemcpyHostToDevice));
    if (!fg.row_depth.empty())
        HIP_TRY(hipMemcpy(b->d_row_depth.p, fg.row_depth.data(), fg.row_depth.size() * 4, hipMemcpyHostToDevice));
    const std::vector<uint32_t>& h_slot = sweep_tables ? g->sweep.slot : fg.d_slot;
    const std::vector<uint32_t>& h_pred_slot = sweep_tables ? g->sweep.pred_slot : fg.pred_dslot;
    if (!h_slot.empty())
        HIP_TRY(hipMemcpy(b->d_dslot.p, h_slot.data(), h_slot.size() * 4, hipMemcpyHostToDevice));
    if (!h_pred_slot.empty())
        HIP_TRY(hipMemcpy(b->d_pred_dslot.p, h_pred_slot.data(), h_pred_slot.size() * 4, hipMemcpyHostToDevice));
    if (sweep) HIP_TRY(hipMemset(b->d_pair_off.p, 0, ((size_t)n_queries + 1) * 8));
    if (qoff[n_queries]) HIP_TRY(hipMemcpy(b->d_qseq.p, qseq, qoff[n_queries], hipMemcpyHostToDevice));
    HIP_TRY(hipMemcpy(b->d_qoff.p, qoff, ((size_t)n_queries + 1) * 8, hipMemcpyHostToDevice));
    HIP_TRY(hipMemcpy(b->d_scratch_off.p, b->h_scratch_off.data(), ((size_t)n_queries + 1) * 8, hipMemcpyHostToDevice));
    if (n_queries) {
        HIP_TRY(hipMemcpy(b->d_pitch.p, b->h_pitch.data(), (size_t)n_queries * 4, hipMemcpyHostToDevice));
        for (int k = 0; k < (b->plan16_same ? 1 : 3); ++k)
            HIP_TRY(hipMemcpy(b->plan[k].d_off.p, b->plan[k].off.data(), (size_t)n_queries * 8, hipMemcpyHostToDevice));
    }
    HIP_TRY(hipEventRecord(e1, nullptr));
    HIP_TRY(hipEventSynchronize(e1));
    (void)hipEventElapsedTime(&b->ms_h2d, e0, e1);
    (void)hipEventDestroy(e0);
    (void)hipEventDestroy(e1);

    *out = b.release();
    return POA_OK;
}

static int prepare_exact(poa_batch* b, const poa_costs_t* costs, const poa_config_t* cfg) {
    const FlatGraph& fg = b->graph->g;
    std::string err;
    int rc;
    {
        std::lock_guard<std::mutex> lk(const_cast<poa_graph*>(b->graph)->bubble_mu);
        rc = build_bubble_index(const_cast<FlatGraph&>(fg), err);
    }
    if (rc != POA_OK) return fail(rc, err);
    const uint32_t n = fg.n;
    {
        uint32_t skew = 0;
        for (uint32_t r = 0; r < n; ++r) skew = std::max<uint32_t>(skew, fg.dist_max[r] - std::min(fg.dist_min[r], fg.dist_max[r]));
        b->ex_skew = skew;
    }
    const uint32_t maxc = std::max<uint32_t>(costs->mismatch, (uint32_t)costs->gap_open + costs->gap_extend);
    const uint64_t n_prio64 = ((uint64_t)n + b->max_len + 2) * maxc + costs->gap_open + ((uint64_t)n + b->max_len) * costs->gap_extend + 64;
    if (n_prio64 > (1ull << 26)) return fail(POA_ERR_UNSUPPORTED, "exact replay: priority range too large for this graph / query size");
    if (3ull * n * (((uint64_t)b->max_len + 64) & ~63ull) >= (1ull << 32))
        return fail(POA_ERR_UNSUPPORTED, "exact replay: the visited table of one query exceeds 2^32 cells");
    if ((uint64_t)fg.n_exit * ((b->max_len + 64) / 64) >= (1ull << 32))
        return fail(POA_ERR_UNSUPPORTED, "exact replay: reached sets of one query exceed 2^32 words");
    const float f = (cfg && cfg->queue_entries_per_cell > 0.f) ? cfg->queue_entries_per_cell : 0.25f;
    const uint64_t pool64 = std::max<uint64_t>(256, (uint64_t)(f * (double)n * (double)(b->max_len + 1)));
    if (pool64 > 0xFFFFFFF0ull) return fail(POA_ERR_UNSUPPORTED, "exact replay: queue pool too large");
    uint32_t win = 64;
    {
        const uint64_t win_need = (uint64_t)maxc + costs->gap_open + ((uint64_t)b->ex_skew + 3) * costs->gap_extend + 8;
        while (win < win_need && win < (1u << 24)) win *= 2;
    }
    const uint64_t pool_ws = pool64 + (uint64_t)BQ_CHUNK * (3ull * win + 8);
    if (pool_ws > 0xFFFFFFF0ull) return fail(POA_ERR_UNSUPPORTED, "exact replay: queue pool too large");
    const uint32_t n_prio = (uint32_t)n_prio64, pool_cap = (uint32_t)pool_ws;
    b->ex_win = win;
    const uint32_t stack_cap = (uint32_t)(n + b->max_len + 8), wpn = (uint32_t)((b->max_len + 1 + 63) / 64), swpn = (wpn + 63) / 64;
    if (b->exact_ready && b->ex_n_prio >= n_prio && b->ex_pool_cap >= pool_cap) return POA_OK;
    if (b->ran) HIP_TRY(hipStreamSynchronize(b->last_stream));
    const uint64_t slots = b->plan[0].max_chunk;
    size_t free_b = 0, total_b = 0;
    HIP_TRY(hipMemGetInfo(&free_b, &total_b));
    const uint64_t need = slots * ((uint64_t)fg.n_exit * (wpn + swpn) * 8 + 3ull * n_prio * 4 + (uint64_t)stack_cap * 12 + (uint64_t)pool_cap * 16);
    if (need + (256ull << 20) > free_b + b->d_ex_pool.n * 16 + b->d_ex_head.n * 4 + b->d_ex_reached.n * 8)
        return fail(POA_ERR_OUT_OF_MEMORY, "exact replay workspace does not fit: create the batch with a smaller workspace_bytes (fewer queries per chunk) or lower queue_entries_per_cell");
    if (!b->exact_ready) {
        HIP_TRY(b->d_succ_off.alloc(fg.succ_row_off.size()));
        HIP_TRY(b->d_succ_rows.alloc(std::max<size_t>(fg.succ_rows.size(), 1)));
        HIP_TRY(b->d_dist_min.alloc(n)); HIP_TRY(b->d_dist_max.alloc(n)); HIP_TRY(b->d_exit_idx.alloc(n));
        HIP_TRY(b->d_node_row.alloc(n)); HIP_TRY(b->d_sp_to_end.alloc(n));
        HIP_TRY(b->d_ex_end.alloc(2 * (size_t)std::max<uint32_t>(b->n_queries, 1)));
        HIP_TRY(hipMemcpy(b->d_node_row.p, fg.node_row.data(), n * 4, hipMemcpyHostToDevice));
        HIP_TRY(hipMemcpy(b->d_sp_to_end.p, fg.sp_to_end.data(), n * 4, hipMemcpyHostToDevice));
        HIP_TRY(b->d_ex_sym.alloc((size_t)n + 4));
        {
            std::vector<uint8_t> row_sym((size_t)n + 4, 0);
            for (uint32_t r = 0; r < n; ++r) row_sym[r] = fg.rows[r].sym;
            HIP_TRY(hipMemcpy(b->d_ex_sym.p, row_sym.data(), row_sym.size(), hipMemcpyHostToDevice));
        }
        HIP_TRY(b->d_nbm_off.alloc(n + 1)); HIP_TRY(b->d_nbm.alloc(std::max<size_t>(fg.nbm.size(), 1)));
        if (!fg.row_rec.empty()) {
            HIP_TRY(b->d_ex_rec.alloc(fg.row_rec.size()));
            HIP_TRY(hipMemcpy(b->d_ex_rec.p, fg.row_rec.data(), fg.row_rec.size() * sizeof(FlatGraph::RowRec), hipMemcpyHostToDevice));
        }
        HIP_TRY(b->d_ex_status.alloc(std::max<uint32_t>(b->n_queries, 1)));
        HIP_TRY(b->d_ex_counters.alloc(4 * (size_t)std::max<uint32_t>(b->n_queries, 1)));
// ... 80 lines not shown
        CkptParams kp;
        kp.rows = b->d_rows.p; kp.pred_rows = b->d_pred_rows.p; kp.slot = b->d_dslot.p; kp.pred_slot = b->d_pred_dslot.p;
        kp.snap_off = b->d_ck_snap_off.p; kp.snap_dst = b->d_ck_snap_dst.p; kp.pred_src = b->d_ck_pred_src.p; kp.boundary = b->d_ck_boundary.p;
        kp.n_rows = fg.n; kp.n_slots = b->ckpt_slots; kp.n_snap = cp.n_snap_rows; kp.seg_rows = cp.max_segment; kp.n_segments = cp.n_segments();
        kp.start_row = fg.start_row; kp.end_row = fg.end_row;
        kp.first_query = ch.first; kp.n_queries = ch.count;
        kp.qseq = b->d_qseq.p; kp.qoff = b->d_qoff.p; kp.pitch = b->d_pitch.p; kp.plane_off = PL.d_off.p;
        kp.planes = b->d_planes.p; kp.carry = b->d_carry.p;
        kp.cost_x = costs->mismatch; kp.cost_o = costs->gap_open; kp.cost_e = costs->gap_extend;
        kp.scratch_off = b->d_scratch_off.p; kp.scratch = b->d_scratch.p;
        kp.score = b->d_score.p; kp.flags = b->d_flags.p; kp.n_pairs = b->d_npairs.p;
        uint32_t max_pitch = 0;
        uint64_t pitch_sum = 0;
        for (uint32_t i = ch.first; i < ch.first + ch.count; ++i) { max_pitch = std::max(max_pitch, b->h_pitch[i]); pitch_sum += b->h_pitch[i]; }
        b->sweep_bytes_written += (2ull * (b->sweep_slotted + cp.n_snap_rows) + 3ull * fg.n) * pitch_sum * (narrow ? 2 : 4);
        const dim3 grid((ch.count + 3) / 4), block(256);
        launch_by_pitch(narrow, max_pitch, [&](auto cell, auto q) {
            hipLaunchKernelGGL((poa_ckpt_sweep_kernel<decltype(q)::value, decltype(cell)>), grid, block, 0, stream, kp);
        });
        HIP_TRY(hipGetLastError());
        if (const int rc = run.mark()) return rc;
        launch_by_pitch(narrow, max_pitch, [&](auto cell, auto q) {
            hipLaunchKernelGGL((poa_ckpt_trace_kernel<decltype(q)::value, decltype(cell)>), grid, block, 0, stream, kp);
        });
        HIP_TRY(hipGetLastError());
        if (const int rc = run.mark(2)) return rc;
    }
    return run.end_pairs();
}

int poa_batch_run(poa_batch_t* b, const poa_costs_t* costs, void* stream_v) { return poa_batch_run_ex(b, costs, nullptr, stream_v); }

int poa_batch_run_ex(poa_batch_t* b, const poa_costs_t* costs, const poa_config_t* cfg, void* stream_v) {
    if (!b || !costs) return fail(POA_ERR_INVALID_ARG, "poa_batch_run: null argument");
    const TuneView T(cfg);
    uint32_t mode = cfg ? cfg->mode : POA_MODE_DENSE;
    if (mode == POA_MODE_CHECKPOINT2) {
        if (b->ckpt2) return fail(POA_ERR_INVALID_ARG, "poa_batch_run_ex: a POA_MODE_CHECKPOINT2 batch runs through poa_batch_run_2piece only");
        return fail(POA_ERR_UNSUPPORTED, "POA_MODE_CHECKPOINT2 is the two-piece model's checkpointed mode: poa_batch_run_2piece / poa_align_batch_2piece_ex");
    }
    if (mode > POA_MODE_CHECKPOINT2) return fail(POA_ERR_INVALID_ARG, "poa_batch_run_ex: unknown mode");
    if (b->ckpt2) return fail(POA_ERR_INVALID_ARG, "poa_batch_run_ex: the batch was created for POA_MODE_CHECKPOINT2 (it runs in that mode through poa_batch_run_2piece only)");
    if (cfg && cfg->span > POA_SPAN_ENDS_FREE) return fail(POA_ERR_INVALID_ARG, "poa_batch_run_ex: unknown alignment span");
    const bool ends_free = cfg && cfg->span == POA_SPAN_ENDS_FREE;
    if (mode == POA_MODE_SCORE) {
        if (ends_free) return fail(POA_ERR_UNSUPPORTED, "score-only mode is Global: an ends-free result is defined by the reference's search");
        if (!b->sweep) return fail(POA_ERR_INVALID_ARG, "poa_batch_run_ex: POA_MODE_SCORE needs a batch created by poa_batch_create_ex with that mode");
        return run_sweep(b, costs->mismatch, costs->gap_open, costs->gap_extend, T, (hipStream_t)stream_v);
    }
    if (mode == POA_MODE_CHECKPOINT) {
        if (ends_free) return fail(POA_ERR_UNSUPPORTED, "checkpointed mode is Global: an ends-free result is defined by the reference's search");
        if (!b->ckpt) return fail(POA_ERR_INVALID_ARG, "poa_batch_run_ex: POA_MODE_CHECKPOINT needs a batch created by poa_batch_create_ex with that mode");
        return run_ckpt(b, costs, T, (hipStream_t)stream_v);
    }
    if (b->sweep) return fail(POA_ERR_INVALID_ARG, "poa_batch_run_ex: the batch was created for POA_MODE_SCORE (it holds no score planes)");
    if (b->ckpt) return fail(POA_ERR_INVALID_ARG, "poa_batch_run_ex: the batch was created for POA_MODE_CHECKPOINT (it holds no full score planes)");
    if (ends_free) {
        if (cfg->qry_free_end.kind > POA_BOUND_EXCLUDED || cfg->graph_free_begin.kind > POA_BOUND_EXCLUDED ||
            cfg->graph_free_end.kind > POA_BOUND_EXCLUDED || cfg->qry_free_begin.kind > POA_BOUND_EXCLUDED)
            return fail(POA_ERR_INVALID_ARG, "poa_batch_run_ex: unknown bound kind");
        mode = POA_MODE_EXACT;
    }
    if (cfg && cfg->heuristic > POA_HEURISTIC_MINGAP) return fail(POA_ERR_INVALID_ARG, "poa_batch_run_ex: unknown heuristic");
    hipStream_t stream = (hipStream_t)stream_v;
    HIP_TRY(hipSetDevice(b->device));
    const FlatGraph& fg = b->graph->g;
    if (mode != POA_MODE_DENSE && b->n_queries) {
        int rc = prepare_exact(b, costs, cfg);
        if (rc != POA_OK) return rc;
    }
    RunFrame run;
    if (const int rc = run.open(b, "poa_batch_run: call poa_batch_stats/fetch at least every 256 runs")) return rc;
    const DenseRunPlan R = plan_dense_run(costs->gap_open, costs->gap_extend, b->max_len, fg.min_path_nodes, mode,
                                          cfg && (cfg->flags & POA_CFG_FULL_PLANES), b->plan16_same, T);
    if (const int rc = run.begin(stream, b->plan[R.plan].chunks.size())) return rc;
    b->prof_on = T.ptr(POA_TUNE_WS_PROF) != nullptr;
    b->last_mode = mode;
    b->two_piece = false;
    set_layout(b, R.narrow, R.compact, R.relative);
    b->launches.clear();
    b->band_used = false; b->band_queries = 0; b->band_min_d = 0; b->band_chunks = 0;
    b->pair_paired = 0; b->pair_single = 0;
    b->narrow_ran = 0; b->narrow_how = 0; b->narrow_chunks = 0;
    b->tb_kernel = POA_TB_KERNEL_NONE; b->tb_lanes = 0; b->tb_depth = 0; b->tb_walks = 0;
    b->active_plan = R.plan;
    const poa_batch::Plan& PL = b->cur();
    if (b->n_queries == 0) return run.end_empty(true);
    if (R.want_band && !PL.chunks.empty()) {
        if (b->d_band_count.n < 3 * PL.chunks.size()) HIP_TRY(b->d_band_count.alloc(3 * PL.chunks.size()));
        HIP_TRY(hipMemsetAsync(b->d_band_count.p, 0, 3 * PL.chunks.size() * 4, stream));
    }
    for (size_t ci = 0; ci < PL.chunks.size(); ++ci) {
        const auto& ch = PL.chunks[ci];
        uint32_t max_pitch = 0;
        for (uint32_t i = ch.first; i < ch.first + ch.count; ++i) max_pitch = std::max(max_pitch, b->h_pitch[i]);
        const DenseChunkPlan C = plan_dense_chunk(R, ch.count, max_pitch, T, compact_plane_elems(fg.n, max_pitch, fg.d_slot.empty() ? fg.n : fg.n_store_d));
        TbParams tp;
        tp.rows = b->d_rows.p; tp.pred_rows = b->d_pred_rows.p; tp.n_rows = fg.n;
        tp.start_row = fg.start_row; tp.end_row = fg.end_row;
        tp.first_query = ch.first; tp.n_queries = ch.count;
        tp.qseq = b->d_qseq.p; tp.qoff = b->d_qoff.p; tp.pitch = b->d_pitch.p; tp.plane_off = PL.d_off.p;
        tp.planes = b->d_planes.p; tp.scratch_off = b->d_scratch_off.p; tp.scratch = b->d_scratch.p;
        tp.score = b->d_score.p; tp.flags = b->d_flags.p; tp.n_pairs = b->d_npairs.p;
        tp.cost_x = costs->mismatch; tp.cost_o = costs->gap_open; tp.cost_e = costs->gap_extend;
        tp.spec_depth = R.spec_depth;
        tp.exact_pass = 0; tp.ex_status = nullptr; tp.ex_end = nullptr; tp.code_fmt = C.v[4];
        tp.row_depth = R.relative ? b->d_row_depth.p : nullptr;
        tp.d_slot = fg.d_slot.empty() ? nullptr : b->d_dslot.p; tp.pred_dslot = fg.d_slot.empty() ? nullptr : b->d_pred_dslot.p;
        FwdParams fp;
        fp.rows = b->d_rows.p; fp.pred_rows = b->d_pred_rows.p; fp.n_rows = fg.n;
        fp.first_query = ch.first; fp.n_queries = ch.count;
        fp.qseq = b->d_qseq.p; fp.qoff = b->d_qoff.p; fp.pitch = b->d_pitch.p; fp.plane_off = PL.d_off.p;
        fp.planes = b->d_planes.p; fp.strip_carry = b->d_carry.p;
        fp.cost_x = costs->mismatch; fp.cost_oe = (uint32_t)costs->gap_open + costs->gap_extend; fp.cost_e = costs->gap_extend;
        fp.cost_de = R.relative ? 0u : fp.cost_e;
        fp.cost_doe = R.relative ? (uint32_t)costs->gap_open : fp.cost_oe;
        fp.cost_ie = R.relative ? 2u * fp.cost_e : fp.cost_e;
        fp.cost_ioe = R.relative ? fp.cost_oe + fp.cost_e : fp.cost_oe;
        fp.pred_k = R.relative ? b->d_pred_k.p : nullptr;
        fp.d_slot = fg.d_slot.empty() ? nullptr : b->d_dslot.p; fp.pred_dslot = fg.d_slot.empty() ? nullptr : b->d_pred_dslot.p;
        fp.pipeline_error = b->d_pipeline_error.p;
        if (C.mf >= 0) b->dense_derived_gaps = C.mf == 3;
        if (C.band) { if (const int rc = launch_band(b, ci, R, fp, stream)) return rc; }
        else launch_forward(R, C, fp, tp, stream);
        HIP_TRY(hipGetLastError());
        if (const int rc = run.mark()) return rc;

        if (C.separate_tb) {
            launch_traceback(R, C, tp, stream);
            HIP_TRY(hipGetLastError());
            if (!C.lean_tb) b->tb_kernel = POA_TB_KERNEL_GENERIC;
            else if (b->tb_kernel == POA_TB_KERNEL_NONE) b->tb_kernel = POA_TB_KERNEL_LEAN;
            b->tb_lanes = C.v[5]; b->tb_depth = C.v[6]; b->tb_walks += C.v[7];
        }
        if (mode == POA_MODE_DENSE) b->launches.push_back(C);
        if (const int rc = run.mark()) return rc;

        if (mode != POA_MODE_DENSE) {
            if (const int rc = replay_chunk(b, ch, costs, cfg, T, mode == POA_MODE_HYBRID ? 1u : 0u, ends_free, tp, stream)) return rc;
        }
        if (const int rc = run.mark()) return rc;
    }
    return run.end_pairs();
}

int poa_batch_fetch(poa_batch_t* b, uint32_t* score, poa_aln_pair_t* pairs, uint64_t* pair_off, uint64_t pair_capacity,
                    uint32_t* flags, poa_stats_t* stats) {
    if (!b) return fail(POA_ERR_INVALID_ARG, "poa_batch_fetch: null batch");
    if (!b->ran) return fail(POA_ERR_INVALID_ARG, "poa_batch_fetch: poa_batch_run has not been called");
    HIP_TRY(hipSetDevice(b->device));
    HIP_TRY(hipStreamSynchronize(b->last_stream));
    {
        int prc = check_pipeline_error(b);
        if (prc != POA_OK) return prc;
    }
    const uint32_t n = b->n_queries;
    hipEvent_t e0, e1;
    HIP_TRY(hipEventCreate(&e0));
    HIP_TRY(hipEventCreate(&e1));
    HIP_TRY(hipEventRecord(e0, nullptr));
    std::vector<uint64_t> off_local;
    uint64_t* off = pair_off;
    if (!off) { off_local.resize((size_t)n + 1); off = off_local.data(); }
    HIP_TRY(hipMemcpy(off, b->d_pair_off.p, ((size_t)n + 1) * 8, hipMemcpyDeviceToHost));
    int rc = POA_OK;
    uint32_t n_exact = 0;
    if (n) {
        if (score) HIP_TRY(hipMemcpy(score, b->d_score.p, (size_t)n * 4, hipMemcpyDeviceToHost));
        std::vector<uint32_t> fl_local;
        uint32_t* fl = flags;
        if (!fl && stats) { fl_local.resize(n); fl = fl_local.data(); }
        if (fl) HIP_TRY(hipMemcpy(fl, b->d_flags.p, (size_t)n * 4, hipMemcpyDeviceToHost));
        if (pairs) {
            if (off[n] > pair_capacity) rc = fail(POA_ERR_CAPACITY, "pair_capacity too small; pair_off[n] holds the needed total");
            else if (off[n]) HIP_TRY(hipMemcpy(pairs, b->d_pairs.p, off[n] * sizeof(poa_aln_pair_t), hipMemcpyDeviceToHost));
        }
        if (stats && fl) {
            uint32_t nf = 0;
            for (uint32_t i = 0; i < n; ++i) nf += fl[i] != 0;
            stats->n_flagged = nf;
        }
        if (stats && (b->last_mode == POA_MODE_EXACT || b->last_mode == POA_MODE_HYBRID)) {
            std::vector<uint32_t> stt(n);
            HIP_TRY(hipMemcpy(stt.data(), b->d_ex_status.p, (size_t)n * 4, hipMemcpyDeviceToHost));
            uint32_t ne = 0;
            for (uint32_t i = 0; i < n; ++i) ne += stt[i] == 0;
            n_exact = ne;
        }
    } else if (stats) {
        stats->n_flagged = 0;
    }
    HIP_TRY(hipEventRecord(e1, nullptr));
    HIP_TRY(hipEventSynchronize(e1));
    float ms_d2h = 0.f;
    (void)hipEventElapsedTime(&ms_d2h, e0, e1);
    (void)hipEventDestroy(e0);
    (void)hipEventDestroy(e1);
    if (stats) {
        collect_stats(b, stats);
        stats->ms_d2h = ms_d2h;
        stats->n_exact = n_exact;
    }
    return rc;
}

int poa_batch_stats(poa_batch_t* b, poa_stats_t* stats) {
    if (!b || !stats) return fail(POA_ERR_INVALID_ARG, "poa_batch_stats: null argument");
    HIP_TRY(hipSetDevice(b->device));
    if (b->ran) HIP_TRY(hipStreamSynchronize(b->last_stream));
    std::memset(stats, 0, sizeof(*stats));
    collect_stats(b, stats);
    return b->ran ? check_pipeline_error(b) : POA_OK;
}

int poa_batch_fetch_search_counters(poa_batch_t* b, uint32_t* out) {
// ... 3 lines not shown
    HIP_TRY(hipSetDevice(b->device));
    HIP_TRY(hipStreamSynchronize(b->last_stream));
    if (b->n_queries) HIP_TRY(hipMemcpy(out, b->d_ex_counters.p, (size_t)b->n_queries * 16, hipMemcpyDeviceToHost));
    if (b->prof_on && b->d_ex_prof.p && b->n_queries) {
        std::vector<unsigned long long> pr(8 * (size_t)b->n_queries);
        HIP_TRY(hipMemcpy(pr.data(), b->d_ex_prof.p, pr.size() * 8, hipMemcpyDeviceToHost));
        unsigned long long sum[8] = {0};
        for (size_t i = 0; i < pr.size(); ++i) sum[i & 7] += pr[i];
        fprintf(stderr, "[ws prof] cycles / counts: %llu %llu %llu %llu %llu %llu %llu %llu\n", sum[0], sum[1], sum[2], sum[3], sum[4], sum[5], sum[6], sum[7]);
    }
    return POA_OK;
}

int poa_batch_device_results(poa_batch_t* b, void** score, void** flags, void** pair_off, void** pairs) {
    if (!b) return fail(POA_ERR_INVALID_ARG, "poa_batch_device_results: null batch");
    if (b->ran) {
        HIP_TRY(hipSetDevice(b->device));
        HIP_TRY(hipStreamSynchronize(b->last_stream));
        const int prc = check_pipeline_error(b);
        if (prc != POA_OK) return prc;
    }
    if (score) *score = b->d_score.p;
    if (flags) *flags = b->d_flags.p;
    if (pair_off) *pair_off = b->d_pair_off.p;
    if (pairs) *pairs = b->d_pairs.p;
    return POA_OK;
}

int poa_batch_last_layout(poa_batch_t* b, uint32_t* layout) {
    if (!b || !layout) return fail(POA_ERR_INVALID_ARG, "poa_batch_last_layout: null argument");
    if (!b->ran) return fail(POA_ERR_INVALID_ARG, "poa_batch_last_layout: poa_batch_run has not been called");
    *layout = (b->dense_narrow ? POA_LAYOUT_U16 : 0u) | (b->dense_compact ? POA_LAYOUT_COMPACT : 0u) | (b->dense_relative ? POA_LAYOUT_RELATIVE : 0u) |
              (b->dense_derived_gaps ? POA_LAYOUT_DERIVED_GAPS : 0u);
    return POA_OK;
}

int poa_batch_last_launch(poa_batch_t* b, uint32_t chunk, uint32_t out[8]) {
    if (!b || !out) return fail(POA_ERR_INVALID_ARG, "poa_batch_last_launch: null argument");
    if (!b->ran) return fail(POA_ERR_INVALID_ARG, "poa_batch_last_launch: poa_batch_run has not been called");
    if (b->two_piece || b->sweep || b->ckpt || b->last_mode != POA_MODE_DENSE)
        return fail(POA_ERR_UNSUPPORTED, "poa_batch_last_launch: the last run was not a dense one-piece run");
    if (chunk >= b->launches.size()) return fail(POA_ERR_INVALID_ARG, "poa_batch_last_launch: the last run had no such chunk");
    for (int k = 0; k < 8; ++k) out[k] = b->launches[chunk].v[k];
    return POA_OK;
}

int poa_batch_band_info(poa_batch_t* b, uint32_t out[4]) {
    if (!b || !out) return fail(POA_ERR_INVALID_ARG, "poa_batch_band_info: null argument");
    if (!b->ran) return fail(POA_ERR_INVALID_ARG, "poa_batch_band_info: poa_batch_run has not been called");
    out[0] = b->band_used ? 1u : 0u; out[1] = 0; out[2] = 0; out[3] = b->band_used ? b->band_min_d : 0u;
    if (!b->band_used) return POA_OK;
    HIP_TRY(hipSetDevice(b->device));
    HIP_TRY(hipStreamSynchronize(b->last_stream));
    std::vector<uint32_t> counts(b->band_chunks);
    HIP_TRY(hipMemcpy(counts.data(), b->d_band_count.p, counts.size() * 4, hipMemcpyDeviceToHost));
    uint32_t fell = 0;
    for (uint32_t c : counts) fell += c;
    out[2] = fell; out[1] = b->band_queries - std::min(fell, b->band_queries);
    return POA_OK;
}

int poa_batch_band_narrow_info(poa_batch_t* b, uint32_t out[4]) {
    if (!b || !out) return fail(POA_ERR_INVALID_ARG, "poa_batch_band_narrow_info: null argument");
    if (!b->ran) return fail(POA_ERR_INVALID_ARG, "poa_batch_band_narrow_info: poa_batch_run has not been called");
    out[0] = b->narrow_ran; out[1] = 0; out[2] = 0; out[3] = b->narrow_how;
    if (!b->narrow_ran) return POA_OK;
    HIP_TRY(hipSetDevice(b->device));
    HIP_TRY(hipStreamSynchronize(b->last_stream));
    const size_t n_chunks = b->cur().chunks.size();
    std::vector<uint32_t> counts(3 * n_chunks);
    HIP_TRY(hipMemcpy(counts.data(), b->d_band_count.p, counts.size() * 4, hipMemcpyDeviceToHost));
    uint32_t missed = 0, missed_both = 0;
    for (size_t c = 0; c < n_chunks; ++c) { missed += counts[n_chunks + c]; missed_both += counts[2 * n_chunks + c]; }
    out[1] = b->narrow_ran - std::min(missed, b->narrow_ran); out[2] = missed - std::min(missed_both, missed);
    return POA_OK;
}

int poa_batch_tb_info(poa_batch_t* b, uint32_t out[4]) {
    if (!b || !out) return fail(POA_ERR_INVALID_ARG, "poa_batch_tb_info: null argument");
    if (!b->ran) return fail(POA_ERR_INVALID_ARG, "poa_batch_tb_info: poa_batch_run has not been called");
    const bool dense_family = !(b->two_piece || b->sweep || b->ckpt);
    out[0] = dense_family ? b->tb_kernel : (uint32_t)POA_TB_KERNEL_NONE;
    out[1] = dense_family ? b->tb_lanes : 0u; out[2] = dense_family ? b->tb_depth : 0u; out[3] = dense_family ? b->tb_walks : 0u;
    return POA_OK;
}

int poa_batch_band_pair_info(poa_batch_t* b, uint32_t out[4]) {
    if (!b || !out) return fail(POA_ERR_INVALID_ARG, "poa_batch_band_pair_info: null argument");
    if (!b->ran) return fail(POA_ERR_INVALID_ARG, "poa_batch_band_pair_info: poa_batch_run has not been called");
    out[0] = b->pair_paired; out[1] = b->pair_single; out[2] = BAND_PAIR_MIN_QUERIES; out[3] = b->pair_paired ? 1u : 0u;
    return POA_OK;
}

int poa_batch_fetch_planes(poa_batch_t* b, uint32_t query, uint32_t* m, uint32_t* i, uint32_t* d) {
    if (!b || !m || !i || !d) return fail(POA_ERR_INVALID_ARG, "poa_batch_fetch_planes: null argument");
    if (!b->ran || query >= b->n_queries) return fail(POA_ERR_INVALID_ARG, "poa_batch_fetch_planes: bad query / not run");
    if (b->compact) return fail(POA_ERR_UNSUPPORTED, "poa_batch_fetch_planes: the last run used the compact layout; run with POA_CFG_FULL_PLANES");
    if (b->sweep) return fail(POA_ERR_UNSUPPORTED, "poa_batch_fetch_planes: a score-only batch keeps no score planes");
    if (b->ckpt) return fail(POA_ERR_UNSUPPORTED, "poa_batch_fetch_planes: a checkpointed batch keeps snapshots and one segment window, no score planes");
    if (b->last_mode != POA_MODE_DENSE) return fail(POA_ERR_UNSUPPORTED, "poa_batch_fetch_planes: after an exact / hybrid run the workspace holds the replayed search's tiled table");
    if (b->two_piece) return fail(POA_ERR_UNSUPPORTED, "poa_batch_fetch_planes: the last run was a two-piece run; its five planes come from poa_batch_fetch_planes_2piece");
    const auto& last = b->cur().chunks.back();
    if (query < last.first || query >= last.first + last.count)
        return fail(POA_ERR_INVALID_ARG, "poa_batch_fetch_planes: the query's planes were overwritten by a later chunk");
    HIP_TRY(hipSetDevice(b->device));
    HIP_TRY(hipStreamSynchronize(b->last_stream));
    const uint32_t rows = b->graph->g.n, pitch = b->h_pitch[query];
    const uint32_t cols = (uint32_t)(b->h_qoff[query + 1] - b->h_qoff[query]) + 1;
    const uint64_t RP = (uint64_t)rows * pitch;
    uint32_t* dst[3] = {m, i, d};
    if (!b->narrow) {
        for (int k = 0; k < 3; ++k) {
            const uint32_t* src = b->d_planes.p + b->cur().off[query] + k * RP;
            HIP_TRY(hipMemcpy2D(dst[k], (size_t)cols * 4, src, (size_t)pitch * 4, (size_t)cols * 4, rows, hipMemcpyDeviceToHost));
        }
    } else {
        std::vector<uint16_t> tmp((size_t)rows * cols);
        const uint16_t* base = reinterpret_cast<const uint16_t*>(b->d_planes.p) + b->cur().off[query];
        for (int k = 0; k < 3; ++k) {
            HIP_TRY(hipMemcpy2D(tmp.data(), (size_t)cols * 2, base + k * RP, (size_t)pitch * 2, (size_t)cols * 2, rows, hipMemcpyDeviceToHost));
            for (size_t t = 0; t < tmp.size(); ++t) dst[k][t] = tmp[t] == 0xFFFFu ? 0xFFFFFFFFu : tmp[t];
        }
    }
    return POA_OK;
}

int poa_batch_fetch_compact(poa_batch_t* b, uint32_t query, uint16_t* m_raw, uint16_t* d, uint8_t* d_kept) {
    if (!b || !m_raw || !d || !d_kept) return fail(POA_ERR_INVALID_ARG, "poa_batch_fetch_compact: null argument");
    if (!b->ran || query >= b->n_queries) return fail(POA_ERR_INVALID_ARG, "poa_batch_fetch_compact: bad query / not run");
    if (b->sweep) return fail(POA_ERR_UNSUPPORTED, "poa_batch_fetch_compact: a score-only batch keeps no score planes");
    if (b->ckpt || b->ckpt2) return fail(POA_ERR_UNSUPPORTED, "poa_batch_fetch_compact: a checkpointed batch keeps snapshots and one segment window, no score planes");
    if (b->last_mode != POA_MODE_DENSE) return fail(POA_ERR_UNSUPPORTED, "poa_batch_fetch_compact: after an exact / hybrid run the workspace holds the replayed search's tiled table");
    if (b->two_piece) return fail(POA_ERR_UNSUPPORTED, "poa_batch_fetch_compact: the last run was a two-piece run; its five planes come from poa_batch_fetch_planes_2piece");
    if (!b->compact || !b->dense_derived_gaps || b->dense_relative)
        return fail(POA_ERR_UNSUPPORTED, "poa_batch_fetch_compact: the last run did not store the compact derived-gaps layout (poa_batch_last_layout)");
    const auto& last = b->cur().chunks.back();
    if (query < last.first || query >= last.first + last.count)
        return fail(POA_ERR_INVALID_ARG, "poa_batch_fetch_compact: the query's planes were overwritten by a later chunk");
    HIP_TRY(hipSetDevice(b->device));
    HIP_TRY(hipStreamSynchronize(b->last_stream));
    const FlatGraph& fg = b->graph->g;
    const uint32_t rows = fg.n, pitch = b->h_pitch[query];
    const uint32_t cols = (uint32_t)(b->h_qoff[query + 1] - b->h_qoff[query]) + 1;
    const uint64_t RP = (uint64_t)rows * pitch;
    const uint16_t* Mp = reinterpret_cast<const uint16_t*>(b->d_planes.p) + b->cur().off[query];
    const uint16_t* Dp = Mp + RP + RP / 4;
    HIP_TRY(hipMemcpy2D(m_raw, (size_t)cols * 2, Mp, (size_t)pitch * 2, (size_t)cols * 2, rows, hipMemcpyDeviceToHost));
    const uint32_t n_slots = fg.d_slot.empty() ? rows : fg.n_store_d;
    std::vector<uint16_t> kept((size_t)n_slots * cols);
    if (n_slots) HIP_TRY(hipMemcpy2D(kept.data(), (size_t)cols * 2, Dp, (size_t)pitch * 2, (size_t)cols * 2, n_slots, hipMemcpyDeviceToHost));
    for (uint32_t r = 0; r < rows; ++r) {
        const uint32_t slot = fg.d_slot.empty() ? r : fg.d_slot[r];
        d_kept[r] = (fg.rows[r].flags & ROW_STORE_D) && slot < n_slots ? 1 : 0;
        if (d_kept[r]) std::copy(kept.begin() + (size_t)slot * cols, kept.begin() + (size_t)(slot + 1) * cols, d + (size_t)r * cols);
        else std::fill(d + (size_t)r * cols, d + (size_t)(r + 1) * cols, (uint16_t)0xFFFFu);
    }
    return POA_OK;
}

static int prepare_two_piece_u32(poa_batch* b) {
    const uint32_t rows = b->graph->g.n, n = b->n_queries;
    uint64_t biggest = 0;
    for (uint32_t i = 0; i < n; ++i) biggest = std::max<uint64_t>(biggest, 5ull * rows * b->h_pitch[i] * 4);
    const uint64_t ws = std::max(b->plan_ws, biggest);
    if (b->d_planes.bytes < ws + 256) {
        if (b->ran) HIP_TRY(hipStreamSynchronize(b->last_stream));
// ... 1106 lines not shown
        fp.pred_k = nullptr;
        fp.d_slot = by_row ? nullptr : m->d_slot.p + gp.row_base; fp.pred_dslot = by_row ? nullptr : m->d_pred_slot.p + gp.edge_base;
        fp.pipeline_error = b->d_pipeline_error.p;
        TbParams& tp = mb.T;
        tp.rows = fp.rows; tp.pred_rows = fp.pred_rows; tp.n_rows = fg.n;
        tp.start_row = fg.start_row; tp.end_row = fg.end_row;
        tp.qseq = fp.qseq; tp.qoff = fp.qoff; tp.pitch = fp.pitch; tp.plane_off = fp.plane_off;
        tp.planes = b->d_planes.p; tp.scratch_off = b->d_scratch_off.p; tp.scratch = b->d_scratch.p;
        tp.score = b->d_score.p; tp.flags = b->d_flags.p; tp.n_pairs = b->d_npairs.p;
        tp.exact_pass = 0; tp.ex_status = nullptr; tp.ex_end = nullptr; tp.code_fmt = 0;
        tp.row_depth = nullptr;
        tp.d_slot = fp.d_slot; tp.pred_dslot = fp.pred_dslot;
        mb.empty = fg.n_real == 0 ? 1u : 0u;
    }

    hipEvent_t e0, e1;
    HIP_TRY(hipEventCreate(&e0));
    HIP_TRY(hipEventCreate(&e1));
    HIP_TRY(hipEventRecord(e0, nullptr));
    auto up = [](void* dst, const void* src, size_t bytes) { return bytes ? hipMemcpy(dst, src, bytes, hipMemcpyHostToDevice) : hipSuccess; };
    HIP_TRY(up(b->d_rows.p, h_rows.data(), h_rows.size() * sizeof(RowMeta)));
    HIP_TRY(up(b->d_pred_rows.p, h_pred_rows.data(), h_pred_rows.size() * 4));
    HIP_TRY(up(m->d_slot.p, h_dslot.data(), h_dslot.size() * 4));
    HIP_TRY(up(m->d_pred_slot.p, h_pred_dslot.data(), h_pred_dslot.size() * 4));
    HIP_TRY(up(m->d_dense.p, h_blocks.data(), h_blocks.size() * sizeof(MultiDenseBlock)));
    HIP_TRY(up(m->d_graph_of.p, pl.graph_of.data(), (size_t)n * 4));
    HIP_TRY(up(b->d_qseq.p, qseq, qoff[n]));
    HIP_TRY(up(b->d_qoff.p, qoff, ((size_t)n + 1) * 8));
    HIP_TRY(up(b->d_scratch_off.p, pl.scratch_off.data(), ((size_t)n + 1) * 8));
    HIP_TRY(up(b->d_pitch.p, pl.pitch.data(), (size_t)n * 4));
    HIP_TRY(up(b->plan[0].d_off.p, pl.region_off.data(), (size_t)n * 8));
    HIP_TRY(hipEventRecord(e1, nullptr));
    HIP_TRY(hipEventSynchronize(e1));
    (void)hipEventElapsedTime(&b->ms_h2d, e0, e1);
    (void)hipEventDestroy(e0);
    (void)hipEventDestroy(e1);

    *out = m.release();
    return POA_OK;
}

int poa_multi_run_dense(poa_multi_t* m, const poa_costs_t* costs, const poa_config_t* cfg, void* stream_v) {
    if (!m || !costs) return fail(POA_ERR_INVALID_ARG, "poa_multi_run_dense: null argument");
    if (!m->dense) return fail(POA_ERR_INVALID_ARG, "poa_multi_run_dense: the batch was not created by poa_multi_create_dense (a checkpointed batch runs through poa_multi_run / poa_multi_run_2piece)");
    const int mrc = multi_dense_mode_check(cfg, "poa_multi_run_dense");
    if (mrc != POA_OK) return mrc;
    const TuneView T(cfg);
    bool narrow = !planes32(T);
    for (size_t g = 0; g < m->ub_open.size(); ++g)
        narrow = narrow && u16_cells_suffice(costs->gap_open, costs->gap_extend, m->ub_open[g], m->ub_extend[g]);
    if (!narrow)
        return fail(POA_ERR_UNSUPPORTED, "poa_multi_run_dense: the run needs u32 cells (the costs' score bound exceeds 65534 for some graph, or "
                                         "tune[POA_TUNE_PLANES] = 32) and a dense multi-graph batch holds u16 compact cells only; the checkpointed "
                                         "batch (poa_multi_create, poa_multi_run) runs either width");
    poa_batch* b = &m->core;
    hipStream_t stream = (hipStream_t)stream_v;
    HIP_TRY(hipSetDevice(b->device));
    RunFrame run;
    if (const int rc = run.open(b, "poa_multi_run_dense: call poa_multi_stats/fetch at least every 256 runs")) return rc;
    const MultiPlan& pl = m->plan;
    if (const int rc = run.begin(stream, pl.chunks.size())) return rc;
    b->last_mode = POA_MODE_DENSE;
    b->two_piece = false;
    set_layout(b, true, true, false);
    b->active_plan = 0;
    b->launches.clear();
    if (b->n_queries == 0) return run.end_empty(true);
    for (const auto& ch : pl.chunks) {
        MultiDenseLaunch ml;
        ml.graphs = m->d_dense.p; ml.graph_of = m->d_graph_of.p;
        ml.first_query = ch.first; ml.n_queries = ch.count;
        ml.cost_x = costs->mismatch; ml.cost_o = costs->gap_open; ml.cost_e = costs->gap_extend;
        ml.spec_depth = 32;
        ml.code_fmt = 0;
        const uint32_t quads = ch.max_pitch <= 512 ? 1u : 2u;
        const dim3 grid((ch.count + 3) / 4), block(256);
        if (quads == 1) hipLaunchKernelGGL((poa_forward_packed_multi_kernel<1>), grid, block, 0, stream, ml);
        else hipLaunchKernelGGL((poa_forward_packed_multi_kernel<2>), grid, block, 0, stream, ml);
        HIP_TRY(hipGetLastError());
        if (const int rc = run.mark()) return rc;
        hipLaunchKernelGGL(poa_traceback_multi_kernel, grid, block, 0, stream, ml);
        HIP_TRY(hipGetLastError());
        if (const int rc = run.mark(2)) return rc;
        b->launches.push_back(DenseChunkPlan{{POA_KERNEL_PACKED, quads, 0u, 4u, ml.code_fmt, 64u, ml.spec_depth, ch.count}, -1, false, true, false});
    }
    return run.end_pairs();
}

int poa_multi_last_launch(poa_multi_t* m, uint32_t chunk, uint32_t out[8]) {
    if (!m || !out) return fail(POA_ERR_INVALID_ARG, "poa_multi_last_launch: null argument");
    if (!m->dense) return fail(POA_ERR_INVALID_ARG, "poa_multi_last_launch: the batch was not created by poa_multi_create_dense");
    if (!m->core.ran) return fail(POA_ERR_INVALID_ARG, "poa_multi_last_launch: poa_multi_run_dense has not been called");
    if (chunk >= m->core.launches.size()) return fail(POA_ERR_INVALID_ARG, "poa_multi_last_launch: the last run had no such chunk");
    for (int k = 0; k < 8; ++k) out[k] = m->core.launches[chunk].v[k];
    return POA_OK;
}

int poa_align_multi_dense(const poa_graph_t* const* graphs, uint32_t n_graphs, const uint64_t* graph_qoff, const poa_costs_t* costs,
                          const poa_config_t* cfg, const uint8_t* qseq, const uint64_t* qoff, uint32_t* score, poa_aln_pair_t* pairs,
                          uint64_t* pair_off, uint64_t pair_capacity, uint32_t* flags, poa_stats_t* stats, int device) {
    if (!costs) return fail(POA_ERR_INVALID_ARG, "poa_align_multi_dense: null argument");
    if (stats) std::memset(stats, 0, sizeof(*stats));
    poa_multi_t* m = nullptr;
    int rc = poa_multi_create_dense(graphs, n_graphs, graph_qoff, device, qseq, qoff, cfg, 0, &m);
    if (rc != POA_OK) return rc;
    rc = poa_multi_run_dense(m, costs, cfg, nullptr);
    if (rc == POA_OK) rc = poa_multi_fetch(m, score, pairs, pair_off, pair_capacity, flags, stats);
    poa_multi_destroy(m);
    return rc;
}

}


struct poa_scoreset {
    poa_batch core;
    ScoreSetPlan plan;
    std::vector<uint64_t> ub_open, ub_extend;
    DevBuf<uint32_t> d_slot, d_pred_slot, d_pair_graph, d_pair_query, d_carry_off, d_class_list[SS_N_VARIANTS];
    DevBuf<ScoreGraphParams> d_params;
    std::vector<uint8_t> cut;
    DevBuf<uint32_t> d_cap, d_swept, d_check_rows;
    uint32_t* h_stage = nullptr;
    hipEvent_t stage_done = nullptr;
    bool stage_busy = false;
    uint32_t check_stride = 0;
    bool last_capped = false;
    DevBuf<unsigned long long> d_best_word;
    DevBuf<uint32_t> d_limit, d_query_off, d_query_pairs, d_best_list[SS_N_VARIANTS];
    DevBuf<ScoreSetBest> d_best;
    bool last_best = false;
    ~poa_scoreset() {
        if (h_stage) (void)hipHostFree(h_stage);
        if (stage_done) (void)hipEventDestroy(stage_done);
    }
};

namespace {
int scoreset_mode_check(const poa_config_t* cfg, const char* who) {
    if (cfg && cfg->mode != POA_MODE_SCORE)
        return fail(POA_ERR_UNSUPPORTED, std::string(who) + ": a score set runs in POA_MODE_SCORE only");
    if (cfg && cfg->span != POA_SPAN_GLOBAL)
        return fail(POA_ERR_UNSUPPORTED, std::string(who) + ": score-only mode is Global: an ends-free result is defined by the reference's search");
    return POA_OK;
}

int scoreset_plan_of(const poa_graph_t* const* graphs, uint32_t n_graphs, uint32_t n_queries, const uint64_t* qoff, uint64_t n_pairs,
                     const uint32_t* pair_query, const uint32_t* pair_graph, uint64_t workspace_bytes, ScoreSetPlan& plan, const char* who) {
    if (!qoff || (n_graphs && !graphs)) return fail(POA_ERR_INVALID_ARG, std::string(who) + ": null argument");
    std::vector<ScoreSetGraphIn> in(n_graphs);
    for (uint32_t g = 0; g < n_graphs; ++g) {
        if (!graphs[g]) return fail(POA_ERR_INVALID_ARG, std::string(who) + ": null graph");
        in[g] = ScoreSetGraphIn{&graphs[g]->g, &graphs[g]->sweep};
    }
    std::string err;
    const int rc = build_scoreset_plan(in.data(), n_graphs, n_queries, qoff, n_pairs, pair_query, pair_graph, workspace_bytes, plan, err);
    if (rc != 0) return fail(rc, std::string(who) + ": " + err);
    return POA_OK;
}

size_t scoreset_stage_front(const poa_scoreset* s) { return std::max<size_t>(s->core.n_queries, s->plan.n_queries); }

int scoreset_cap_buffers(poa_scoreset* s) {
    const size_t n = s->core.n_queries, n_rows = s->plan.n_rows_total;
    if (!s->d_cap.p) HIP_TRY(s->d_cap.alloc(std::max<size_t>(n, 1)));
    if (!s->d_swept.p) HIP_TRY(s->d_swept.alloc(std::max<size_t>(n, 1)));
    if (!s->d_check_rows.p) HIP_TRY(s->d_check_rows.alloc(std::max<size_t>(n_rows, 1)));
// ... 537 lines not shown
```

poasta_amd/csrc/poa_traceback_mf.hpp:

```cpp
#pragma once
#include "poa_kernels.hpp"

namespace poa_amd {

struct MfCtx {
    const RowMeta* rows;
    const uint32_t* pred_rows;
    const uint16_t* M;
    const uint16_t* D;
    const uint32_t* d_slot;
    const uint32_t* pred_dslot;
    const uint8_t* q;
    uint32_t L, pitch, x, o, e;
    __device__ __forceinline__ uint32_t raw(uint32_t row, uint32_t j) const { return (uint32_t)M[row * pitch + j]; }
    __device__ __forceinline__ void cell(uint32_t row, uint32_t j, uint32_t& v, uint32_t& a, uint32_t& cf) const {
        const uint32_t r = raw(row, j);
        v = mf_value(r); a = (r >> 14) & 1u; cf = (r >> 15) & 1u;
    }
    __device__ __forceinline__ uint32_t m(uint32_t row, uint32_t j) const { return mf_value(raw(row, j)); }
    __device__ __forceinline__ uint32_t d_at(uint32_t slot, uint32_t j) const { return PlaneIO<uint16_t>::widen((uint32_t)D[slot * pitch + j]); }
    __device__ __forceinline__ uint32_t d_kept(uint32_t row, uint32_t j) const { return d_at(d_slot ? d_slot[row] : row, j); }
    __device__ __forceinline__ uint32_t pred(uint32_t k) const { return pred_rows[k]; }
    __device__ __forceinline__ uint32_t pred_d(uint32_t k, uint32_t j) const { return d_at(pred_dslot ? pred_dslot[k] : pred_rows[k], j); }
};
// ... 6 lines not shown
    const uint32_t r = a - b;
    if (r == INF) panic = true;
    return r;
}

template <bool END>
__device__ __forceinline__ TbStep mf_step_m(const MfCtx& c, const RowMeta& m, uint32_t row, uint32_t j, uint32_t raw, uint32_t up,
                                            uint32_t& n_cand, bool& panic) {
    TbStep f{0, 0, 0, false, 0, m.node};
    n_cand = 0;
    const uint32_t cs = mf_value(raw);
    f.cs = cs;
    if (cs == INF) return f;
    if (j > 0) {
        const bool moe = END || (uint32_t)m.sym == (uint32_t)c.q[j - 1];
        const uint32_t pj = END ? j : j - 1;
        const uint32_t target = (moe || m.pred_count == 0) ? cs : mf_sub(cs, c.x, panic);
        if (!END && (m.flags & ROW_CHAIN)) {
            if (up == target) mf_cand(f, n_cand, row - 1, pj, 0);
        } else {
            for (uint32_t k = 0; k < m.pred_count; ++k) {
                const uint32_t pr = c.pred_rows[m.pred_begin + k];
                if (c.m(pr, pj) == target) mf_cand(f, n_cand, pr, pj, 0);
            }
        }
    }
    if (raw & 0x8000u) mf_cand(f, n_cand, row, j, 1);
    if (raw & 0x4000u) mf_cand(f, n_cand, row, j, 2);
    return f;
}
__device__ __forceinline__ void mf_load_m(const MfCtx& c, uint32_t row, uint32_t j, uint32_t& raw, uint32_t& up) {
    const uint32_t off = row * c.pitch + j;
    raw = (uint32_t)c.M[off];
    up = (row > 0 && j > 0) ? mf_value((uint32_t)c.M[off - c.pitch - 1u]) : INF;
}

template <bool END>
__device__ __forceinline__ TbStep mf_step_d(const MfCtx& c, const RowMeta& m, uint32_t row, uint32_t j, uint32_t cs, uint32_t above,
                                            uint32_t& n_cand, bool& bad, bool& panic) {
    TbStep f{0, 0, 0, false, cs, m.node};
    n_cand = 0;
    if (cs == INF) return f;
    if (m.pred_count == 0) return f;
    const uint32_t t_open = mf_sub(mf_sub(cs, c.o, panic), c.e, panic), t_ext = mf_sub(cs, c.e, panic);
    const bool is_end = END || (m.flags & ROW_END) != 0;
    const bool real_open = !is_end && (j >= c.L || (uint32_t)m.sym != (uint32_t)c.q[j]);
    if (m.flags & ROW_CHAIN) {
        const uint32_t v = above;
        if (v == t_open) mf_cand(f, n_cand, row - 1, j, 0);
        else if (!real_open && v < t_open) bad = true;
        if (tbd_d_extends(c, row, j, cs)) mf_cand(f, n_cand, row - 1, j, 1);
    } else {
        for (uint32_t k = 0; k < m.pred_count; ++k) {
            const uint32_t pr = c.pred_rows[m.pred_begin + k];
            const uint32_t v = c.m(pr, j);
            if (v == t_open) mf_cand(f, n_cand, pr, j, 0);
            else if (!real_open && v < t_open) bad = true;
        }
        for (uint32_t k = 0; k < m.pred_count; ++k)
            if (c.pred_d(m.pred_begin + k, j) == t_ext) mf_cand(f, n_cand, c.pred_rows[m.pred_begin + k], j, 1);
    }
    return f;
}

__device__ __forceinline__ TbStep mf_step_i(const MfCtx& c, const RowMeta& m, uint32_t row, uint32_t j, uint32_t cs, uint32_t& n_cand,
                                            bool& bad, bool& panic) {
    TbStep f{0, 0, 0, false, cs, m.node};
    n_cand = 0;
    if (cs == INF) return f;
    if (j > 0) {
        const uint32_t t_open = mf_sub(mf_sub(cs, c.o, panic), c.e, panic), t_ext = mf_sub(cs, c.e, panic);
        const uint32_t pm = c.m(row, j - 1);
        if (pm == t_open) mf_cand(f, n_cand, row, j - 1, 0);
        else if (!tbd_open_i(c, m, j - 1) && pm < t_open) bad = true;
        if (tbd_i_extends(c, m, row, j, cs)) {
            const bool only = (n_cand == 0);
            mf_cand(f, n_cand, row, j - 1, 0);
            if (only && pm != t_ext) bad = true;
        }
    }
    return f;
}

template <int GW>
__device__ __forceinline__ void traceback_mf_walk(const TbParams& P, const uint32_t qi, const uint32_t lane) {
    const uint32_t gbase = (threadIdx.x & 63u) - lane;
    auto gballot = [&](bool pred) -> uint64_t {
        const uint64_t b = __ballot(pred);
        if (GW == 64) return b;
        const uint32_t w = (gbase & 32u) ? (uint32_t)(b >> 32) : (uint32_t)b;
        return (uint64_t)((w >> (gbase & 31u)) & (uint32_t)((1ull << (GW & 63)) - 1ull));
    };
    auto ones = [](uint64_t b) -> uint32_t { return (b == ~0ull) ? 64u : (uint32_t)__builtin_ctzll(~b); };
    auto bc = [&](uint32_t v, uint32_t src) { return (uint32_t)__shfl((int)v, (int)(gbase + src)); };

    const uint64_t qbeg = P.qoff[qi];
    MfCtx c;
    c.rows = P.rows; c.pred_rows = P.pred_rows;
    c.L = (uint32_t)(P.qoff[qi + 1] - qbeg);
    c.q = P.qseq + qbeg;
    c.pitch = P.pitch[qi];
    const uint64_t RP = (uint64_t)P.n_rows * c.pitch;
    c.M = reinterpret_cast<const uint16_t*>(P.planes) + P.plane_off[qi];
    c.D = c.M + RP + RP / 4;
    c.d_slot = P.d_slot; c.pred_dslot = P.pred_dslot;
    c.x = P.cost_x; c.o = P.cost_o; c.e = P.cost_e;
    const uint32_t L = c.L, start_row = P.start_row, end_row = P.end_row;

    uint2* out = P.scratch + P.scratch_off[qi];
    const uint32_t cap = (uint32_t)(P.scratch_off[qi + 1] - P.scratch_off[qi]);
    uint32_t cnt = 0;
    uint32_t flags = 0;
    uint32_t lflags = 0;
    auto emit_at = [&](uint32_t pos, uint32_t rpos, uint32_t qpos) {
        if (pos < cap) out[cap - 1 - pos] = make_uint2(rpos, qpos);
    };

    if (lane == 0) P.score[qi] = c.m(end_row, L);
    const uint32_t end_node = c.rows[end_row].node;

    bool done = false;
    uint32_t crow = 0, cj = 0, cst = 0;
    uint32_t gcs = INF;
    if (L == 0) done = true;
    if (!done && L == 1) {
        flags |= POA_FLAG_SHORT_QUERY;
        if (lane == 0) emit_at(0, end_node, 0);
        cnt = 1;
        done = true;
    }
    if (!done) {
        uint32_t f0 = 0, fr = 0, fj = 0, fs = 0, fallback = 0, fg = INF;
        if (lane == 0) {
            uint32_t nc; bool bad = false, pn = false;
            const RowMeta me = c.rows[end_row];
            TbStep cur = mf_step_m<true>(c, me, end_row, L, c.raw(end_row, L), INF, nc, pn);
            fg = cur.cs;
            if (cur.found && !pn && nc != 1) f0 |= POA_FLAG_AMBIGUOUS;
            if (!cur.found && !pn) {
                cur = mf_step_d<true>(c, me, end_row, L, c.d_kept(end_row, L), end_row > 0 ? c.m(end_row - 1, L) : INF, nc, bad, pn);
                fg = cur.cs;
                if (!pn) {
                    if (!cur.found) { f0 |= POA_FLAG_REF_PANIC; fallback = 1; }
                    else f0 |= POA_FLAG_AMBIGUOUS;
                    if (cur.found && cur.st == 1) fg = cur.cs - c.e;
                }
            }
            if (pn) { f0 |= POA_FLAG_REF_PANIC; fallback = 2; }
            fr = cur.row; fj = cur.j; fs = cur.st;
        }
        flags |= bc(f0, 0);
        const uint32_t fb = bc(fallback, 0);
        if (fb) {
            if (fb == 2) flags |= POA_FLAG_TRUNCATED;
            if (fb == 1 && L <= 3) {
                if (lane == 0) for (uint32_t i = 0; i < L; ++i) emit_at(i, end_node, L - 1 - i);
                cnt = L;
            }
            done = true;
        } else {
            crow = bc(fr, 0); cj = bc(fj, 0); cst = bc(fs, 0); gcs = bc(fg, 0);
        }
    }
    bool reached_start = done;
    uint32_t d_run = 0, i_run = 0;
    const uint32_t max_depth = P.spec_depth < (uint32_t)GW ? P.spec_depth : (uint32_t)GW;
    while (!done) {
        uint32_t depth = 1;
        if (cst == 2 && crow != start_row && max_depth > 1 && cj > 1) {
            uint32_t idepth = i_run < max_depth ? (i_run ? i_run : 1u) : max_depth;
            if (idepth < 2) idepth = 2;
            if (cj < idepth) idepth = cj;
            const bool iact = lane < idepth;
            const uint32_t jj = cj - lane;
            TbStep sI{0, 0, 0, false, 0, 0}, sM{0, 0, 0, false, 0, 0};
            uint32_t ncI = 0, ncM = 0;
            bool badI = false, pnI = false, pnM = false;
            RowMeta mi{};
            if (iact) {
                mi = c.rows[crow];
                uint32_t rawL, upL;
                mf_load_m(c, crow, jj - 1, rawL, upL);
                const uint32_t gcs_i = lane == 0 ? gcs : c.m(crow, jj);
                sI = mf_step_i(c, mi, crow, jj, gcs_i, ncI, badI, pnI);
                if (sI.found && !pnI) sM = mf_step_m<false>(c, mi, crow, sI.j, rawL, upL, ncM, pnM);
            }
            const bool cyc = iact && sI.found && !pnI && sI.j + 1 == jj && sM.found && !pnM && sM.st == 2 && sM.row == crow && sM.j == sI.j;
            const uint32_t ip = ones(gballot(cyc));
            if (ip > 0) {
                if (lane < ip) {
                    if (ncI != 1 || badI || ncM != 1) lflags |= POA_FLAG_AMBIGUOUS;
                    if (sI.j == 0 && (uint32_t)mi.sym == (uint32_t)c.q[0]) lflags |= POA_FLAG_START_QUIRK;
                    emit_at(cnt + lane, POA_NONE, jj - 1);
                }
                cnt += ip;
                cj -= ip;
                gcs = bc(sM.cs, ip - 1);
                i_run += ip;
                continue;
            }
            const uint32_t w0 = bc(((sI.found && !pnI) ? 1u : 0u) | ((ncI != 1 || badI) ? 2u : 0u), 0);
            if (w0 & 1u) {
                if (w0 & 2u) flags |= POA_FLAG_AMBIGUOUS;
                if (lane == 0) emit_at(cnt, POA_NONE, cj - 1);
                cnt += 1;
                const uint32_t n_row = crow, n_j = bc(sI.j, 0);
                if (n_j == 0 && (uint32_t)c.rows[n_row].sym == (uint32_t)c.q[0]) flags |= POA_FLAG_START_QUIRK;
                cj = n_j; cst = 0;
                i_run = 0;
                continue;
            }
        }
        if (cst != 2) i_run = 0;
        if (cst == 0) {
            depth = max_depth;
            if (crow + 1 < depth) depth = crow + 1;
            if (cj + 1 < depth) depth = cj + 1;
        } else if (cst == 1) {
            depth = d_run < max_depth ? (d_run ? d_run : 1u) : max_depth;
            if (crow + 1 < depth) depth = crow + 1;
        }
        if (cst != 1) d_run = 0;
        const bool active = lane < depth;
        const uint32_t my_row = crow - lane, my_j = (cst == 0) ? cj - lane : cj;
        TbStep bt{0, 0, 0, false, 0, 0};
        uint32_t nc = 0;
        bool bad = false, pn = false;
        if (active) {
            const RowMeta m = c.rows[my_row];
            if (cst == 0) {
                uint32_t raw, up;
                mf_load_m(c, my_row, my_j, raw, up);
                bt = mf_step_m<false>(c, m, my_row, my_j, raw, up, nc, pn);
            } else if (cst == 1) {
                const uint32_t above = my_row > 0 ? c.m(my_row - 1, my_j) : INF;
                bt = mf_step_d<false>(c, m, my_row, my_j, gcs - lane * c.e, above, nc, bad, pn);
            } else bt = mf_step_i(c, m, my_row, my_j, gcs, nc, bad, pn);
        }
        const bool amb = active && bt.found && (nc != 1 || bad);
        const bool quirk = active && bt.found && bt.st == 0 && bt.j == 0 && bt.row != start_row && cst != 1 &&
                           (uint32_t)c.rows[bt.row].sym == (uint32_t)c.q[0];
        const bool regular = active && bt.found && bt.row + 1 == my_row && bt.row != start_row &&
                             ((cst == 0 && bt.st == 0 && bt.j + 1 == my_j) || (cst == 1 && bt.st == 1 && bt.j == my_j));
        uint32_t p = ones(gballot(regular));
        bool dies = false;
        if (__ballot(active && pn)) {
            const uint64_t pnb = gballot(active && pn);
            const uint32_t first_pn = pnb ? (uint32_t)__builtin_ctzll(pnb) : 64u;
            dies = pnb != 0 && first_pn <= p;
            if (dies) p = first_pn;
        }
        if (lane < p) {
            if (amb) lflags |= POA_FLAG_AMBIGUOUS;
            if (quirk) lflags |= POA_FLAG_START_QUIRK;
            emit_at(cnt + lane, bt.node, cst == 0 ? my_j - 1 : POA_NONE);
        }
        cnt += p;
        if (dies) {
            flags |= POA_FLAG_REF_PANIC;
            break;
        }
        if (p == depth) {
            crow -= depth;
            if (cst == 0) cj -= depth;
            else { gcs -= depth * c.e; d_run += depth; }
            continue;
        }
        const uint32_t dw = bc((bt.found ? 1u : 0u) | (amb ? 2u : 0u) | (quirk ? 4u : 0u) | (bt.st << 3), p);
        const uint32_t d_row = bc(bt.row, p), d_j = bc(bt.j, p), d_cs = bc(bt.cs, p), d_node = bc(bt.node, p);
        const uint32_t d_st = dw >> 3;
        const uint32_t cur_j = (cst == 0) ? cj - p : cj, cur_st = cst;
        if (!(dw & 1u)) break;
        if (dw & 2u) flags |= POA_FLAG_AMBIGUOUS;
        if (cur_st == 0 && d_st != 0) {
            crow = d_row; cj = d_j; cst = d_st;
            gcs = d_cs;
            continue;
        }
        if (lane == 0) {
            if (cur_st == 0) emit_at(cnt, d_node, cur_j - 1);
            else if (cur_st == 2) emit_at(cnt, POA_NONE, cur_j - 1);
            else emit_at(cnt, d_node, POA_NONE);
        }
        cnt += 1;
        if (dw & 4u) flags |= POA_FLAG_START_QUIRK;
        if (d_row == start_row) { reached_start = true; break; }
        if (cur_st == 1 && d_st == 1) gcs = d_cs - c.e;
        if (cur_st == 1) d_run += p + 1;
        crow = d_row; cj = d_j; cst = d_st;
    }
    if (!reached_start) flags |= POA_FLAG_TRUNCATED;
    if (gballot((lflags & POA_FLAG_AMBIGUOUS) != 0)) flags |= POA_FLAG_AMBIGUOUS;
    if (gballot((lflags & POA_FLAG_START_QUIRK) != 0)) flags |= POA_FLAG_START_QUIRK;
    if (lane == 0) {
        P.flags[qi] = flags;
        P.n_pairs[qi] = cnt < cap ? cnt : cap;
    }
}

template <int GW>
__global__ __launch_bounds__(256) void poa_traceback_mf_kernel(TbParams P) {
    const uint32_t lane = threadIdx.x & (uint32_t)(GW - 1);
    const uint32_t wq = (blockIdx.x * blockDim.x + threadIdx.x) / (uint32_t)GW;
    if (wq >= P.n_queries) return;
    traceback_mf_walk<GW>(P, P.first_query + wq, lane);
}

}
```

Measured before the change: 2924.

## Add ancestor spine table for speculative lean traceback along graph predecessors

```diff
diff --git a/include/poasta_amd.h b/include/poasta_amd.h
--- a/include/poasta_amd.h
+++ b/include/poasta_amd.h
@@ -281,4 +281,5 @@
 #include "poasta_amd_scoreset_best.h"
 #include "poasta_amd_tb.h"
 #include "poasta_amd_multi_dense.h"
+#include "poasta_amd_tb_spine.h"
 #endif
diff --git a/include/poasta_amd_tb_spine.h b/include/poasta_amd_tb_spine.h
--- /dev/null
+++ b/include/poasta_amd_tb_spine.h
@@ -0,0 +1,19 @@
+#ifndef POASTA_AMD_TB_SPINE_H
+#define POASTA_AMD_TB_SPINE_H
+#include "poasta_amd.h"
+#ifdef __cplusplus
+extern "C" {
+#endif
+
+#define POA_TB_SPINE_SHIFT 6
+enum {
+    POA_TB_SPINE_OFF = 0,
+    POA_TB_SPINE_PLAIN,
+    POA_TB_SPINE_PATCH
+};
+int poa_batch_tb_spine_info(poa_batch_t* b, uint32_t out[2]);
+
+#ifdef __cplusplus
+}
+#endif
+#endif
diff --git a/poasta_amd/_lib.py b/poasta_amd/_lib.py
--- a/poasta_amd/_lib.py
+++ b/poasta_amd/_lib.py
@@ -32,6 +32,8 @@
 CFG_BEST_PAIR_ORDER = 2
 EXPORTS_TB = ["poa_batch_tb_info"]
 TB_LEAN_SHIFT = 4
+EXPORTS_TB_SPINE = ["poa_batch_tb_spine_info"]
+TB_SPINE_SHIFT = 6
 EXPORTS_MULTI_DENSE = ["poa_multi_footprint_dense", "poa_multi_create_dense", "poa_multi_run_dense", "poa_align_multi_dense",
                        "poa_graph_compact_elems", "poa_multi_last_launch"]
 
@@ -81,6 +83,10 @@
     if lv is not None and lv != "":
         i = TUNE_KEYS.index("BAND_PAIR")
         vals[i] = (vals[i] if i in vals else 2) | ((2 if int(lv) else 1) << TB_LEAN_SHIFT)
+    sv = overrides.get("tb_spine", os.environ.get("POA_TB_SPINE"))
+    if sv is not None and sv != "":
+        i = TUNE_KEYS.index("BAND_PAIR")
+        vals[i] = (vals[i] if i in vals else 2) | ((int(sv) & 3) << TB_SPINE_SHIFT)
     if cfg is None:
         if not vals:
             return None
@@ -117,7 +123,7 @@
 
 
 def build(force=False):
-    srcs = [os.path.join(CSRC, f) for f in os.listdir(CSRC)] + [os.path.join(_HERE, "..", "include", h) for h in ("poasta_amd.h", "poasta_amd_scoreset_cap.h", "poasta_amd_scoreset_best.h", "poasta_amd_tb.h", "poasta_amd_multi_dense.h")]
+    srcs = [os.path.join(CSRC, f) for f in os.listdir(CSRC)] + [os.path.join(_HERE, "..", "include", h) for h in ("poasta_amd.h", "poasta_amd_scoreset_cap.h", "poasta_amd_scoreset_best.h", "poasta_amd_tb.h", "poasta_amd_multi_dense.h", "poasta_amd_tb_spine.h")]
     stale = not os.path.exists(LIB_PATH) or any(os.path.getmtime(s) > os.path.getmtime(LIB_PATH) for s in srcs)
     if force or stale:
         subprocess.check_call(["make", "-C", CSRC] + (["-B"] if force else []))
@@ -221,6 +227,9 @@
     if hasattr(L, "poa_batch_tb_info"):
         L.poa_batch_tb_info.restype = C.c_int
         L.poa_batch_tb_info.argtypes = [vp, vp]
+    if hasattr(L, "poa_batch_tb_spine_info"):
+        L.poa_batch_tb_spine_info.restype = C.c_int
+        L.poa_batch_tb_spine_info.argtypes = [vp, vp]
     if hasattr(L, "poa_batch_last_launch"):
         L.poa_batch_last_launch.restype = C.c_int
         L.poa_batch_last_launch.argtypes = [vp, C.c_uint32, vp]
diff --git a/poasta_amd/aligner.py b/poasta_amd/aligner.py
--- a/poasta_amd/aligner.py
+++ b/poasta_amd/aligner.py
@@ -356,6 +356,11 @@
         out = (C.c_uint32 * 4)()
         _lib.check(_lib.lib().poa_batch_tb_info(self.handle, out))
         return {"kernel": (None, "generic", "lean")[int(out[0])], "lanes": int(out[1]), "depth": int(out[2]), "walks": int(out[3])}
+
+    def tb_spine_info(self):
+        out = (C.c_uint32 * 2)()
+        _lib.check(_lib.lib().poa_batch_tb_spine_info(self.handle, out))
+        return {"variant": (None, "spine", "patch")[int(out[0])], "table_bytes": int(out[1])}
 
     def launches(self):
         out = []
diff --git a/poasta_amd/csrc/poa_dense_plan.cpp b/poasta_amd/csrc/poa_dense_plan.cpp
--- a/poasta_amd/csrc/poa_dense_plan.cpp
+++ b/poasta_amd/csrc/poa_dense_plan.cpp
@@ -1,4 +1,6 @@
 #include "poa_dense_plan.hpp"
+
+#include "../../include/poasta_amd_tb_spine.h"
 
 #include <algorithm>
 
@@ -52,11 +54,14 @@
     R.band_pair = -1;
     R.band_narrow = -1;
     R.tb_lean = -1;
+    R.tb_spine = -1;
     if (const int* pv = T.ptr(POA_TUNE_BAND_PAIR)) {
         const int p = (*pv) & POA_BAND_PAIR_MASK, n = ((*pv) >> POA_BAND_NARROW_SHIFT) & 3, l = ((*pv) >> POA_TB_LEAN_SHIFT) & 3;
         if (p != POA_BAND_PAIR_RULE) R.band_pair = p != 0 ? 1 : 0;
         if (n) R.band_narrow = n - 1;
         if (l == 1 || l == 2) R.tb_lean = l - 1;
+        const int s = ((*pv) >> POA_TB_SPINE_SHIFT) & 3;
+        if (s) R.tb_spine = s - 1;
     }
     R.tb_lean_mode = mode == POA_MODE_DENSE;
     return R;
@@ -64,6 +69,12 @@
 
 bool tb_lean_eligible(const DenseRunPlan& R, uint32_t tb_lanes, uint32_t code_fmt, uint64_t plane_elems) {
     return R.tb_lean_mode && tb_lanes != 0 && R.compact && code_fmt == 4 && !R.relative && plane_elems < (1ull << 32);
+}
+
+constexpr int POA_TB_SPINE_RULE_VARIANT = POA_TB_SPINE_PATCH;
+int tb_spine_variant(const DenseRunPlan& R, bool lean, bool have_spine, uint32_t depth) {
+    if (!lean || !have_spine || depth > 32 || R.tb_spine == 0) return POA_TB_SPINE_OFF;
+    return R.tb_spine < 0 ? POA_TB_SPINE_RULE_VARIANT : R.tb_spine;
 }
 
 constexpr uint32_t BAND_NARROW_MIN_SHARE = 4;
@@ -77,7 +88,8 @@
     return pair_by_rule ? n_rule : 0;
 }
 
-DenseChunkPlan plan_dense_chunk(const DenseRunPlan& R, uint32_t count, uint32_t max_pitch, const TuneView& T, uint64_t plane_elems) {
+DenseChunkPlan plan_dense_chunk(const DenseRunPlan& R, uint32_t count, uint32_t max_pitch, const TuneView& T, uint64_t plane_elems,
+                                bool have_spine) {
     uint32_t lk = POA_KERNEL_NONE, lq = 0, lwaves = 4, code_fmt = 0;
     bool lfuse = false, lmw = false;
     int mf = -1;
@@ -128,7 +140,8 @@
         if (R.compact && !T.ptr(POA_TUNE_TB_DEPTH)) ldepth = tbg == 16 ? 16u : 32u;
     }
     const bool lean = R.tb_lean != 0 && tb_lean_eligible(R, ltb, code_fmt, plane_elems);
-    return {{lk, lq, (lfuse ? POA_LAUNCH_FUSE : 0u) | (lmw ? POA_LAUNCH_MW : 0u), lwaves, code_fmt, ltb, ldepth, count}, mf, lk == POA_KERNEL_BAND, ltb != 0, lean};
+    return {{lk, lq, (lfuse ? POA_LAUNCH_FUSE : 0u) | (lmw ? POA_LAUNCH_MW : 0u), lwaves, code_fmt, ltb, ldepth, count}, mf, lk == POA_KERNEL_BAND, ltb != 0, lean,
+            tb_spine_variant(R, lean, have_spine, ldepth)};
 }
 
 }
diff --git a/poasta_amd/csrc/poa_dense_plan.hpp b/poasta_amd/csrc/poa_dense_plan.hpp
--- a/poasta_amd/csrc/poa_dense_plan.hpp
+++ b/poasta_amd/csrc/poa_dense_plan.hpp
@@ -27,6 +27,7 @@
     uint32_t band_cap, spec_depth;
     int tb_lean;
     bool tb_lean_mode;
+    int tb_spine;
 };
 DenseRunPlan plan_dense_run(uint32_t gap_open, uint32_t gap_extend, uint64_t max_len, uint64_t min_path_nodes, uint32_t mode, bool full_planes,
                             bool plan16_same, const TuneView& T);
@@ -37,9 +38,12 @@
     bool band;
     bool separate_tb;
     bool lean_tb;
+    int spine_tb;
 };
-DenseChunkPlan plan_dense_chunk(const DenseRunPlan& R, uint32_t count, uint32_t max_pitch, const TuneView& T, uint64_t plane_elems = ~0ull);
+DenseChunkPlan plan_dense_chunk(const DenseRunPlan& R, uint32_t count, uint32_t max_pitch, const TuneView& T, uint64_t plane_elems = ~0ull,
+                                bool have_spine = false);
 bool tb_lean_eligible(const DenseRunPlan& R, uint32_t tb_lanes, uint32_t code_fmt, uint64_t plane_elems);
+int tb_spine_variant(const DenseRunPlan& R, bool lean, bool have_spine, uint32_t depth);
 uint32_t band_narrow_class(uint32_t d_n, uint32_t L);
 uint32_t band_narrow_pairs(const DenseRunPlan& R, bool pair_by_rule, uint32_t n_rule, uint32_t n_any);
 }
diff --git a/poasta_amd/csrc/poa_engine.hip b/poasta_amd/csrc/poa_engine.hip
--- a/poasta_amd/csrc/poa_engine.hip
+++ b/poasta_amd/csrc/poa_engine.hip
@@ -20,6 +20,7 @@
 #include "poa_fsearch.hpp"
 
 #include "poa_dense_plan.hpp"
+#include "poa_tb_spine.hpp"
 #include "poa_kernels.hpp"
 #include "poa_traceback_mf.hpp"
 #include "poa_forward_packed.hpp"
@@ -248,6 +249,9 @@
     std::vector<uint32_t> h_band_nnarrow_rule, h_band_nnarrow_any;
     uint32_t narrow_ran = 0, narrow_how = 0, narrow_chunks = 0;
     uint32_t tb_kernel = 0, tb_lanes = 0, tb_depth = 0, tb_walks = 0;
+    DevBuf<uint32_t> d_tb_spine;
+    uint64_t tb_spine_table_bytes = 0;
+    int tb_spine = -1;
     int band_pair_plan = -1;
     std::vector<uint32_t> h_band_npair;
     DevBuf<uint32_t> d_band_order;
@@ -621,12 +625,21 @@
     return POA_OK;
 }
 
-void launch_traceback(const DenseRunPlan& R, const DenseChunkPlan& c, const TbParams& tp, hipStream_t stream) {
+template <int SPINE>
+void launch_traceback_spine(uint32_t lanes, dim3 grid, dim3 block, const TbSpineParams& sp, hipStream_t stream) {
+    if (lanes == 16) hipLaunchKernelGGL((poa_traceback_mf_spine_kernel<16, SPINE>), grid, block, 0, stream, sp);
+    else if (lanes == 32) hipLaunchKernelGGL((poa_traceback_mf_spine_kernel<32, SPINE>), grid, block, 0, stream, sp);
+    else if (lanes == 8) hipLaunchKernelGGL((poa_traceback_mf_spine_kernel<8, SPINE>), grid, block, 0, stream, sp);
+    else hipLaunchKernelGGL((poa_traceback_mf_spine_kernel<64, SPINE>), grid, block, 0, stream, sp);
+}
+void launch_traceback(const DenseRunPlan& R, const DenseChunkPlan& c, const TbParams& tp, const uint32_t* spine, hipStream_t stream) {
     const uint32_t lanes = c.v[5], per_block = 256 / lanes;
     const dim3 grid((c.v[7] + per_block - 1) / per_block), block(256);
     TbParams tpg = tp;
     tpg.spec_depth = c.v[6];
-    if (c.lean_tb && lanes == 16) hipLaunchKernelGGL((poa_traceback_mf_kernel<16>), grid, block, 0, stream, tpg);
+    if (c.lean_tb && c.spine_tb == POA_TB_SPINE_PATCH) launch_traceback_spine<2>(lanes, grid, block, TbSpineParams{tpg, spine}, stream);
+    else if (c.lean_tb && c.spine_tb == POA_TB_SPINE_PLAIN) launch_traceback_spine<1>(lanes, grid, block, TbSpineParams{tpg, spine}, stream);
+    else if (c.lean_tb && lanes == 16) hipLaunchKernelGGL((poa_traceback_mf_kernel<16>), grid, block, 0, stream, tpg);
     else if (c.lean_tb && lanes == 32) hipLaunchKernelGGL((poa_traceback_mf_kernel<32>), grid, block, 0, stream, tpg);
     else if (c.lean_tb && lanes == 8) hipLaunchKernelGGL((poa_traceback_mf_kernel<8>), grid, block, 0, stream, tpg);
     else if (c.lean_tb) hipLaunchKernelGGL((poa_traceback_mf_kernel<64>), grid, block, 0, stream, tpg);
@@ -1089,6 +1102,11 @@
     const bool sweep_tables = sweep || ckpt;
     HIP_TRY(b->d_dslot.alloc(std::max<size_t>(sweep_tables ? g->sweep.slot.size() : fg.d_slot.size(), 1)));
     HIP_TRY(b->d_pred_dslot.alloc(std::max<size_t>(sweep_tables ? g->sweep.pred_slot.size() : fg.pred_dslot.size(), 1)));
+    std::vector<uint32_t> h_spine;
+    if (!sweep_tables && n_queries && build_tb_spine(fg.rows, fg.pred_rows, h_spine)) {
+        HIP_TRY(b->d_tb_spine.alloc(h_spine.size()));
+        b->tb_spine_table_bytes = tb_spine_bytes(fg.rows.size());
+    }
     if (ckpt) {
         const CheckpointPlan& cp = b->ckpt_plan;
         HIP_TRY(b->d_ck_snap_off.alloc(cp.snap_off.size()));
@@ -1136,6 +1154,8 @@
         HIP_TRY(hipMemcpy(b->d_dslot.p, h_slot.data(), h_slot.size() * 4, hipMemcpyHostToDevice));
     if (!h_pred_slot.empty())
         HIP_TRY(hipMemcpy(b->d_pred_dslot.p, h_pred_slot.data(), h_pred_slot.size() * 4, hipMemcpyHostToDevice));
+    if (!h_spine.empty())
+        HIP_TRY(hipMemcpy(b->d_tb_spine.p, h_spine.data(), h_spine.size() * 4, hipMemcpyHostToDevice));
     if (sweep) HIP_TRY(hipMemset(b->d_pair_off.p, 0, ((size_t)n_queries + 1) * 8));
     if (qoff[n_queries]) HIP_TRY(hipMemcpy(b->d_qseq.p, qseq, qoff[n_queries], hipMemcpyHostToDevice));
     HIP_TRY(hipMemcpy(b->d_qoff.p, qoff, ((size_t)n_queries + 1) * 8, hipMemcpyHostToDevice));
@@ -1382,7 +1402,7 @@
     b->band_used = false; b->band_queries = 0; b->band_min_d = 0; b->band_chunks = 0;
     b->pair_paired = 0; b->pair_single = 0;
     b->narrow_ran = 0; b->narrow_how = 0; b->narrow_chunks = 0;
-    b->tb_kernel = POA_TB_KERNEL_NONE; b->tb_lanes = 0; b->tb_depth = 0; b->tb_walks = 0;
+    b->tb_kernel = POA_TB_KERNEL_NONE; b->tb_lanes = 0; b->tb_depth = 0; b->tb_walks = 0; b->tb_spine = -1;
     b->active_plan = R.plan;
     const poa_batch::Plan& PL = b->cur();
     if (b->n_queries == 0) return run.end_empty(true);
@@ -1394,7 +1414,8 @@
         const auto& ch = PL.chunks[ci];
         uint32_t max_pitch = 0;
         for (uint32_t i = ch.first; i < ch.first + ch.count; ++i) max_pitch = std::max(max_pitch, b->h_pitch[i]);
-        const DenseChunkPlan C = plan_dense_chunk(R, ch.count, max_pitch, T, compact_plane_elems(fg.n, max_pitch, fg.d_slot.empty() ? fg.n : fg.n_store_d));
+        const DenseChunkPlan C = plan_dense_chunk(R, ch.count, max_pitch, T, compact_plane_elems(fg.n, max_pitch, fg.d_slot.empty() ? fg.n : fg.n_store_d),
+                                                  b->d_tb_spine.p != nullptr && b->tb_spine_table_bytes != 0);
         TbParams tp;
         tp.rows = b->d_rows.p; tp.pred_rows = b->d_pred_rows.p; tp.n_rows = fg.n;
         tp.start_row = fg.start_row; tp.end_row = fg.end_row;
@@ -1427,10 +1448,12 @@
         if (const int rc = run.mark()) return rc;
 
         if (C.separate_tb) {
-            launch_traceback(R, C, tp, stream);
+            launch_traceback(R, C, tp, b->d_tb_spine.p, stream);
             HIP_TRY(hipGetLastError());
             if (!C.lean_tb) b->tb_kernel = POA_TB_KERNEL_GENERIC;
             else if (b->tb_kernel == POA_TB_KERNEL_NONE) b->tb_kernel = POA_TB_KERNEL_LEAN;
+            const int variant = C.lean_tb ? C.spine_tb : (int)POA_TB_SPINE_OFF;
+            b->tb_spine = b->tb_spine < 0 ? variant : (b->tb_spine == variant ? variant : (int)POA_TB_SPINE_OFF);
             b->tb_lanes = C.v[5]; b->tb_depth = C.v[6]; b->tb_walks += C.v[7];
         }
         if (mode == POA_MODE_DENSE) b->launches.push_back(C);
@@ -1600,6 +1623,15 @@
     const bool dense_family = !(b->two_piece || b->sweep || b->ckpt);
     out[0] = dense_family ? b->tb_kernel : (uint32_t)POA_TB_KERNEL_NONE;
     out[1] = dense_family ? b->tb_lanes : 0u; out[2] = dense_family ? b->tb_depth : 0u; out[3] = dense_family ? b->tb_walks : 0u;
+    return POA_OK;
+}
+
+int poa_batch_tb_spine_info(poa_batch_t* b, uint32_t out[2]) {
+    if (!b || !out) return fail(POA_ERR_INVALID_ARG, "poa_batch_tb_spine_info: null argument");
+    if (!b->ran) return fail(POA_ERR_INVALID_ARG, "poa_batch_tb_spine_info: poa_batch_run has not been called");
+    const bool dense_family = !(b->two_piece || b->sweep || b->ckpt);
+    out[0] = dense_family && b->tb_spine > 0 ? (uint32_t)b->tb_spine : (uint32_t)POA_TB_SPINE_OFF;
+    out[1] = (uint32_t)b->tb_spine_table_bytes;
     return POA_OK;
 }
 
@@ -2872,7 +2904,7 @@
         hipLaunchKernelGGL(poa_traceback_multi_kernel, grid, block, 0, stream, ml);
         HIP_TRY(hipGetLastError());
         if (const int rc = run.mark(2)) return rc;
-        b->launches.push_back(DenseChunkPlan{{POA_KERNEL_PACKED, quads, 0u, 4u, ml.code_fmt, 64u, ml.spec_depth, ch.count}, -1, false, true, false});
+        b->launches.push_back(DenseChunkPlan{{POA_KERNEL_PACKED, quads, 0u, 4u, ml.code_fmt, 64u, ml.spec_depth, ch.count}, -1, false, true, false, 0});
     }
     return run.end_pairs();
 }
diff --git a/poasta_amd/csrc/poa_tb_spine.cpp b/poasta_amd/csrc/poa_tb_spine.cpp
--- /dev/null
+++ b/poasta_amd/csrc/poa_tb_spine.cpp
@@ -0,0 +1,27 @@
+#include "poa_tb_spine.hpp"
+
+namespace poa_amd {
+
+uint64_t tb_spine_bytes(uint64_t n_rows) { return n_rows * TB_SPINE_STRIDE * 4ull; }
+
+bool build_tb_spine(const std::vector<RowMeta>& rows, const std::vector<uint32_t>& pred_rows, std::vector<uint32_t>& anc) {
+    anc.clear();
+    const uint64_t n = rows.size();
+    if (n == 0 || tb_spine_bytes(n) > TB_SPINE_MAX_BYTES) return false;
+    for (uint64_t r = 0; r < n; ++r) {
+        const RowMeta& m = rows[r];
+        if (m.pred_count == 0) continue;
+        if ((uint64_t)m.pred_begin + m.pred_count > pred_rows.size() || pred_rows[m.pred_begin] >= r) return false;
+    }
+    anc.assign(n * TB_SPINE_STRIDE, TB_SPINE_NONE);
+    for (uint64_t r = 0; r < n; ++r) {
+        uint32_t* a = anc.data() + r * TB_SPINE_STRIDE;
+        a[0] = (uint32_t)r;
+        if (rows[r].pred_count == 0) continue;
+        const uint32_t* pa = anc.data() + (uint64_t)pred_rows[rows[r].pred_begin] * TB_SPINE_STRIDE;
+        for (uint32_t i = 0; i < TB_SPINE_DEPTH; ++i) a[i + 1] = pa[i];
+    }
+    return true;
+}
+
+}
diff --git a/poasta_amd/csrc/poa_tb_spine.hpp b/poasta_amd/csrc/poa_tb_spine.hpp
--- /dev/null
+++ b/poasta_amd/csrc/poa_tb_spine.hpp
@@ -0,0 +1,15 @@
+#pragma once
+#include <cstdint>
+#include <vector>
+
+#include "poa_graph.hpp"
+
+namespace poa_amd {
+constexpr uint32_t TB_SPINE_DEPTH = 32;
+constexpr uint32_t TB_SPINE_STRIDE = TB_SPINE_DEPTH + 1;
+constexpr uint32_t TB_SPINE_NONE = 0xFFFFFFFFu;
+constexpr uint64_t TB_SPINE_MAX_BYTES = 64ull << 20;
+
+uint64_t tb_spine_bytes(uint64_t n_rows);
+bool build_tb_spine(const std::vector<RowMeta>& rows, const std::vector<uint32_t>& pred_rows, std::vector<uint32_t>& anc);
+}
diff --git a/poasta_amd/csrc/poa_traceback_mf.hpp b/poasta_amd/csrc/poa_traceback_mf.hpp
--- a/poasta_amd/csrc/poa_traceback_mf.hpp
+++ b/poasta_amd/csrc/poa_traceback_mf.hpp
@@ -112,8 +112,14 @@
     return f;
 }
 
-template <int GW>
-__device__ __forceinline__ void traceback_mf_walk(const TbParams& P, const uint32_t qi, const uint32_t lane) {
+struct TbSpineParams {
+    TbParams P;
+    const uint32_t* anc;
+};
+constexpr uint32_t MF_SPINE_STRIDE = 33, MF_SPINE_NONE = 0xFFFFFFFFu;
+
+template <int GW, int SPINE = 0>
+__device__ __forceinline__ void traceback_mf_walk(const TbParams& P, const uint32_t qi, const uint32_t lane, const uint32_t* anc = nullptr) {
     const uint32_t gbase = (threadIdx.x & 63u) - lane;
     auto gballot = [&](bool pred) -> uint64_t {
         const uint64_t b = __ballot(pred);
@@ -194,7 +200,9 @@
     }
     bool reached_start = done;
     uint32_t d_run = 0, i_run = 0;
-    const uint32_t max_depth = P.spec_depth < (uint32_t)GW ? P.spec_depth : (uint32_t)GW;
+    uint32_t max_depth_ = P.spec_depth < (uint32_t)GW ? P.spec_depth : (uint32_t)GW;
+    if (SPINE != 0 && max_depth_ > MF_SPINE_STRIDE - 1) max_depth_ = MF_SPINE_STRIDE - 1;
+    const uint32_t max_depth = max_depth_;
     while (!done) {
         uint32_t depth = 1;
         if (cst == 2 && crow != start_row && max_depth > 1 && cj > 1) {
@@ -244,15 +252,23 @@
         if (cst != 2) i_run = 0;
         if (cst == 0) {
             depth = max_depth;
-            if (crow + 1 < depth) depth = crow + 1;
+            if (SPINE == 0 && crow + 1 < depth) depth = crow + 1;
             if (cj + 1 < depth) depth = cj + 1;
         } else if (cst == 1) {
             depth = d_run < max_depth ? (d_run ? d_run : 1u) : max_depth;
-            if (crow + 1 < depth) depth = crow + 1;
+            if (SPINE == 0 && crow + 1 < depth) depth = crow + 1;
         }
         if (cst != 1) d_run = 0;
-        const bool active = lane < depth;
-        const uint32_t my_row = crow - lane, my_j = (cst == 0) ? cj - lane : cj;
+        bool active = lane < depth;
+        uint32_t my_row = crow - lane, next = 0;
+        const uint32_t my_j = (cst == 0) ? cj - lane : cj;
+        if constexpr (SPINE != 0) {
+            if (active && cst != 2) {
+                const uint32_t* a = anc + crow * MF_SPINE_STRIDE + lane;
+                my_row = a[0]; next = a[1];
+                active = my_row != MF_SPINE_NONE;
+            }
+        }
         TbStep bt{0, 0, 0, false, 0, 0};
         uint32_t nc = 0;
         bool bad = false, pn = false;
@@ -270,12 +286,14 @@
         const bool amb = active && bt.found && (nc != 1 || bad);
         const bool quirk = active && bt.found && bt.st == 0 && bt.j == 0 && bt.row != start_row && cst != 1 &&
                            (uint32_t)c.rows[bt.row].sym == (uint32_t)c.q[0];
-        const bool regular = active && bt.found && bt.row + 1 == my_row && bt.row != start_row &&
+        const bool regular = active && bt.found && (SPINE != 0 ? bt.row == next : bt.row + 1 == my_row) && bt.row != start_row &&
                              ((cst == 0 && bt.st == 0 && bt.j + 1 == my_j) || (cst == 1 && bt.st == 1 && bt.j == my_j));
-        uint32_t p = ones(gballot(regular));
+        const uint64_t regb = gballot(regular);
+        uint32_t p = ones(regb);
         bool dies = false;
+        uint64_t pnb = 0;
         if (__ballot(active && pn)) {
-            const uint64_t pnb = gballot(active && pn);
+            pnb = gballot(active && pn);
             const uint32_t first_pn = pnb ? (uint32_t)__builtin_ctzll(pnb) : 64u;
             dies = pnb != 0 && first_pn <= p;
             if (dies) p = first_pn;
@@ -286,12 +304,40 @@
             emit_at(cnt + lane, bt.node, cst == 0 ? my_j - 1 : POA_NONE);
         }
         cnt += p;
+        if constexpr (SPINE == 2) {
+            const bool off_spine = active && cst == 0 && bt.found && bt.st == 0 && bt.j + 1 == my_j && bt.row != next && bt.row != start_row;
+            while (pnb == 0 && p + 2 < depth) {
+                if (!bc(off_spine ? 1u : 0u, p)) break;
+                const uint32_t d_row = bc(bt.row, p), a2 = bc(my_row, p + 2), d_j = cj - p - 1;
+                if (a2 == MF_SPINE_NONE || a2 == start_row) break;
+                const RowMeta m2 = c.rows[d_row];
+                const uint32_t raw2 = c.raw(d_row, d_j), cand2 = c.m(a2, d_j - 1), cs2 = mf_value(raw2);
+                if (m2.pred_count != 1 || cs2 == INF) break;
+                if (((m2.flags & ROW_CHAIN) ? d_row - 1 : c.pred_rows[m2.pred_begin]) != a2) break;
+                bool pn2 = false;
+                const uint32_t target2 = (uint32_t)m2.sym == (uint32_t)c.q[d_j - 1] ? cs2 : mf_sub(cs2, c.x, pn2);
+                if (pn2 || cand2 != target2) break;
+                if (raw2 & 0xC000u) flags |= POA_FLAG_AMBIGUOUS;
+                if (d_j == 1 && (uint32_t)c.rows[a2].sym == (uint32_t)c.q[0]) flags |= POA_FLAG_START_QUIRK;
+                if (lane == 0) emit_at(cnt + 1, m2.node, d_j - 1);
+                const uint32_t from = p + 2;
+                const uint32_t q2 = from + ones(regb >> from);
+                if (lane == p || (lane >= from && lane < q2)) {
+                    if (amb) lflags |= POA_FLAG_AMBIGUOUS;
+                    if (quirk) lflags |= POA_FLAG_START_QUIRK;
+                    emit_at(cnt + lane - p, bt.node, my_j - 1);
+                }
+                cnt += q2 - p;
+                p = q2;
+            }
+        }
         if (dies) {
             flags |= POA_FLAG_REF_PANIC;
             break;
         }
         if (p == depth) {
-            crow -= depth;
+            if constexpr (SPINE != 0) crow = bc(next, depth - 1);
+            else crow -= depth;
             if (cst == 0) cj -= depth;
             else { gcs -= depth * c.e; d_run += depth; }
             continue;
@@ -336,4 +382,13 @@
     traceback_mf_walk<GW>(P, P.first_query + wq, lane);
 }
 
-}
+template <int GW, int SPINE>
+__global__ __launch_bounds__(256) __attribute__((amdgpu_waves_per_eu(GW <= 16 && SPINE == 2 ? 7 : 1))) void poa_traceback_mf_spine_kernel(TbSpineParams S) {
+    static_assert(SPINE == 1 || SPINE == 2, "the kernel of SPINE 0 is poa_traceback_mf_kernel");
+    const uint32_t lane = threadIdx.x & (uint32_t)(GW - 1);
+    const uint32_t wq = (blockIdx.x * blockDim.x + threadIdx.x) / (uint32_t)GW;
+    if (wq >= S.P.n_queries) return;
+    traceback_mf_walk<GW, SPINE>(S.P, S.P.first_query + wq, lane, S.anc);
+}
+
+}
```

Measured after the change: 2423. 0.829x the previous value.
